# DaviGuanabara/dronechase

Measured on AMD Instinct MI355X. Metric: env-steps/sec (whole job), random-action rollout, higher is better.
Workload: dtype f32

## Files before the change

dronechase_amd/csrc/te_engage.hpp:

```cpp
#pragma once
#include "te_logic.hpp"
#include "te_stacked.hpp"
#include <type_traits>

namespace te {

#if defined(TE_DEBUG_STAMPS) && !defined(TE_NO_ESTAMP)
#define TE_ESTAMP(idx, wait)                                                                                   \
  do {                                                                                                         \
    if (wait) asm volatile("s_waitcnt vmcnt(0) lgkmcnt(0)" ::: "memory");                                      \
    if (p.dbg && threadIdx.x == 0) p.dbg[64 + blockIdx.x * 16 + (idx)] = __builtin_amdgcn_s_memrealtime();     \
  } while (0)
#else
#define TE_ESTAMP(idx, wait) do {} while (0)
#endif

template <class V> TE_DEV void plan_slot_l4(uint16_t* __restrict__ items, int dense_min, int lane, int s, bool a, uint64_t& dense, int& n, uint64_t& live) {
  const unsigned long long b = __ballot(a);
  const int cnt = __popcll(b);
  if (cnt == 0) return;
  live |= (uint64_t)1 << s;
  if (s == 0 || cnt >= dense_min || n + cnt > kMixedCap) { dense |= (uint64_t)1 << s; return; }
  if (a) items[n + (int)__builtin_amdgcn_mbcnt_hi((uint32_t)(b >> 32), __builtin_amdgcn_mbcnt_lo((uint32_t)b, 0u))] = (uint16_t)(lane | (s << 8));
  n += cnt;
// ... 137 lines not shown
    }
    if (invader || reset) st(TE_D_NAV_STATE, s, (uint32_t)TE_NAV_WAIT);
    return respawn;
  }
};

template <int DM>
TE_DEV void drone_contact_pass(const Params& p, int env, bool valid, uint64_t A) {
  const te_config& c = p.cfg;
  const int D = p.D;
  const EnvIO io(p, env);
  float qx[DM], qy[DM], qz[DM], ux[DM], uy[DM], uz[DM];
  uint64_t moved = 0u;
#pragma unroll
  for (int s = 0; s < DM; ++s) {
    qx[s] = qy[s] = qz[s] = ux[s] = uy[s] = uz[s] = 0.0f;
    if (s < D) {
      qx[s] = io.ldf(TE_D_POS, s); qy[s] = io.ldf(TE_D_POS + 1, s); qz[s] = io.ldf(TE_D_POS + 2, s);
      ux[s] = io.ldf(TE_D_VEL, s); uy[s] = io.ldf(TE_D_VEL + 1, s); uz[s] = io.ldf(TE_D_VEL + 2, s);
    }
  }
  const float two_r = 2.0f * c.contact_radius;
#pragma unroll
  for (int i = 0; i < DM; ++i) {
#pragma unroll
    for (int j = i + 1; j < DM; ++j) {
      float nx = qx[j] - qx[i], ny = qy[j] - qy[i], nz = qz[j] - qz[i];
      const float d = sqrtf(nx * nx + ny * ny + nz * nz);
      const bool hit = valid && ((A >> i) & (A >> j) & 1u) != 0u && d < two_r && d > 0.0f;
      const float inv = hit ? 1.0f / d : 0.0f;
      nx *= inv; ny *= inv; nz *= inv;
      const float push = hit ? 0.5f * (two_r - d) : 0.0f;
      const float vn = (ux[j] - ux[i]) * nx + (uy[j] - uy[i]) * ny + (uz[j] - uz[i]) * nz;
      const float dv = (hit && vn < 0.0f) ? 0.5f * vn : 0.0f;
      qx[i] -= push * nx; qy[i] -= push * ny; qz[i] -= push * nz; qx[j] += push * nx; qy[j] += push * ny; qz[j] += push * nz;
      ux[i] += dv * nx; uy[i] += dv * ny; uz[i] += dv * nz; ux[j] -= dv * nx; uy[j] -= dv * ny; uz[j] -= dv * nz;
      moved |= hit ? (((uint64_t)1 << i) | ((uint64_t)1 << j)) : (uint64_t)0;
    }
  }
#pragma unroll
  for (int s = 0; s < DM; ++s) {
    if ((moved >> s) & 1u) {
      io.stf(TE_D_POS, s, qx[s]); io.stf(TE_D_POS + 1, s, qy[s]); io.stf(TE_D_POS + 2, s, qz[s]);
      io.stf(TE_D_VEL, s, ux[s]); io.stf(TE_D_VEL + 1, s, uy[s]); io.stf(TE_D_VEL + 2, s, uz[s]);
    }
  }
}

template <int PM, int IM, bool CONTACT = false>
__global__ __launch_bounds__(64) void engage_kernel(Params p, const float* __restrict__ actions, StepOut o) {
  TE_EXACT
  constexpr int DM = PM + IM;
  using M = typename std::conditional<(DM > 32), uint64_t, uint32_t>::type;
  constexpr M one = 1;
  auto popc = [](M m) { return sizeof(M) == 8 ? __popcll((unsigned long long)m) : __popc((uint32_t)m); };
  auto lowest = [](M m) { return sizeof(M) == 8 ? __ffsll((long long)m) - 1 : __ffs((int)(uint32_t)m) - 1; };
  __shared__ float xs[DM][4];
  __shared__ float rows[64 * TE_OBS_INERTIAL_WORDS];
  const te_config& c = p.cfg;
  const int D = p.D, P = c.n_pursuers;
  const int lane = threadIdx.x;
  const int env = blockIdx.x * 64 + lane;
  const bool valid = env < p.N;
  const GView g{p.dstate, p.estate, D, p.Npad, env, P};
  TE_ESTAMP(0, 0);
  const M pur_bits = (one << P) - one, all_bits = D >= (int)(8 * sizeof(M)) ? ~(M)0 : ((one << D) - one), inv_bits = all_bits & ~pur_bits;
  const bool scripted = all_scripted(c);

  const __amdgpu_buffer_rsrc_t rd = __builtin_amdgcn_make_buffer_rsrc(p.dstate, 0, (int)((uint32_t)(TE_DRONE_WORDS + TE_X_WORDS) * (uint32_t)D * (uint32_t)p.Npad * 4u), 0x00020000);
  const __amdgpu_buffer_rsrc_t re = __builtin_amdgcn_make_buffer_rsrc(p.estate, 0, (int)((uint32_t)TE_ENV_WORDS * (uint32_t)p.Npad * 4u), 0x00020000);
  const int voff = env * 4;
  const uint32_t plane = (uint32_t)p.Npad * 4u;
  auto ld = [&](int w, int s) { return __builtin_amdgcn_raw_buffer_load_b32(rd, voff, (int)(((uint32_t)w * (uint32_t)D + (uint32_t)s) * plane), 0); };
  auto le = [&](int w) { return __builtin_amdgcn_raw_buffer_load_b32(re, voff, (int)((uint32_t)w * plane), 0); };
  auto st = [&](int w, int s, uint32_t v) { __builtin_amdgcn_raw_buffer_store_b32(v, rd, voff, (int)(((uint32_t)w * (uint32_t)D + (uint32_t)s) * plane), 0); };
  auto stf = [&](int w, int s, float v) { st(w, s, __float_as_uint(v)); };
  auto stv = [&](int w, int slot_off, uint32_t v) { __builtin_amdgcn_raw_buffer_store_b32(v, rd, slot_off, (int)((uint32_t)w * (uint32_t)D * plane), 0); };
  auto ste = [&](int w, uint32_t v) { __builtin_amdgcn_raw_buffer_store_b32(v, re, voff, (int)((uint32_t)w * plane), 0); };
  auto stef = [&](int w, float v) { ste(w, __float_as_uint(v)); };
  float px[DM], py[DM], pz[DM];
  uint32_t armed_w[DM];
  int mun[PM], lf[PM];
  float fx[PM], fy[PM], fz[PM];
  const uint32_t* __restrict__ lm32 = reinterpret_cast<const uint32_t*>(p.live_mask);
  const uint64_t live = (uint64_t)__builtin_amdgcn_readfirstlane(lm32[2 * blockIdx.x]) | ((uint64_t)__builtin_amdgcn_readfirstlane(lm32[2 * blockIdx.x + 1]) << 32);
#pragma unroll
  for (int s = 0; s < DM; ++s) {
    px[s] = py[s] = pz[s] = 0.0f; armed_w[s] = 0u;
    if (s < D && (s < P || ((live >> s) & 1u))) {
      px[s] = __uint_as_float(ld(TE_D_OBS_POS, s)); py[s] = __uint_as_float(ld(TE_D_OBS_POS + 1, s)); pz[s] = __uint_as_float(ld(TE_D_OBS_POS + 2, s));
      armed_w[s] = ld(TE_D_ARMED, s);
    }
  }
#pragma unroll
  for (int q = 0; q < PM; ++q) {
    mun[q] = 0; lf[q] = 0; fx[q] = fy[q] = fz[q] = 0.0f;
    if (q < P) {
      mun[q] = (int)ld(TE_D_MUNITION, q); lf[q] = (int)ld(TE_D_LAST_FIRED, q);
      fx[q] = __uint_as_float(ld(TE_D_FORMATION, q)); fy[q] = __uint_as_float(ld(TE_D_FORMATION + 1, q)); fz[q] = __uint_as_float(ld(TE_D_FORMATION + 2, q));
    }
  }
  float ag[9];
#pragma unroll
  for (int k = 0; k < 9; ++k) ag[k] = __uint_as_float(ld(TE_D_OBS_EULER + k, 0));
  uint32_t se[3][PM];
#pragma unroll
  for (int k = 0; k < 3; ++k)
#pragma unroll
    for (int q = 0; q < PM; ++q) se[k][q] = (p.snap && q < P) ? ld(TE_D_OBS_EULER + k, q) : 0u;
  int step = (int)le(TE_E_STEP) + 1;
  int max_step = (int)le(TE_E_MAX_STEP);
  int round = (int)le(TE_E_ROUND);
  const float last_dist = __uint_as_float(le(TE_E_LAST_DIST));
  int agent_kills = (int)le(TE_E_AGENT_KILLS), allies_kills = (int)le(TE_E_ALLIES_KILLS), deads = (int)le(TE_E_DEADS);
  uint32_t episode = le(TE_E_EPISODE);
  float4 act = make_float4(0.0f, 0.0f, 0.0f, 0.0f);
  if (valid) act = reinterpret_cast<const float4*>(actions)[env];

  TE_ESTAMP(1, 1);
  M S = 0, zone = 0, org = 0;
#pragma unroll
  for (int s = 0; s < DM; ++s) {
    const M a = (s < D && armed_w[s] != 0u && valid) ? one : (M)0;
    const float n = fnorm(V3{px[s], py[s], pz[s]});
    S |= a << s;
    zone |= (a & (n > c.dome_radius ? one : (M)0)) << s;
    org |= (a & (n < c.origin_range ? one : (M)0)) << s;
  }
  int tgt[PM]; float dmin[PM];
#pragma unroll
  for (int q = 0; q < PM; ++q) {
    tgt[q] = -1; dmin[q] = 0.0f;
#pragma unroll
    for (int j = 1; j < DM; ++j) {
      const float d = fdist(V3{px[q], py[q], pz[q]}, V3{px[j], py[j], pz[j]});
      const bool take = q < P && j >= P && ((S >> q) & (S >> j) & one) != 0 && (tgt[q] < 0 || d < dmin[q]);
      tgt[q] = take ? j : tgt[q];
      dmin[q] = take ? d : dmin[q];
    }
  }
  auto pos_of = [&](int s) {
    V3 r{0.0f, 0.0f, 0.0f};
#pragma unroll
    for (int k = 0; k < DM; ++k) if (k == s) r = V3{px[k], py[k], pz[k]};
    return r;
  };

  TE_ESTAMP(2, 0);
  M A = S;
  if (valid) {
    stef(TE_E_LAST_ACTION + 0, act.x); stef(TE_E_LAST_ACTION + 1, act.y); stef(TE_E_LAST_ACTION + 2, act.z); stef(TE_E_LAST_ACTION + 3, act.w);
    ste(TE_E_STEP, (uint32_t)step);
    ste(TE_E_SNAP_MASK, (uint32_t)S); ste(TE_E_SNAP_MASK_HI, (uint32_t)((uint64_t)S >> 32));
  }
  M killed = 0;
  auto kill = [&](int j) { killed |= one << j; A &= ~(one << j); };
  int agent_shots = 0, ally_shots = 0, exploded = 0, pursuer_suicided = 0, agent_suicided = 0;
#pragma unroll
  for (int q = 0; q < PM; ++q) {
    if (q < P && valid && ((S >> q) & one) && tgt[q] >= 0 && dmin[q] < c.shoot_range && gun_available(c, mun[q], lf[q], step) && mun[q] > 0) {
      mun[q] -= 1; lf[q] = step;
      st(TE_D_MUNITION, q, (uint32_t)mun[q]); st(TE_D_LAST_FIRED, q, (uint32_t)step);
      const U4 r = env_rng(c, env, RNG_HIT, (uint32_t)q, 0, episode, (uint32_t)step);
      if (u01(r.x) < c.hit_prob) {
        kill(tgt[q]);
        if (q == 0) agent_shots += 1; else ally_shots += 1;
        if (c.evaluation) g.si(TE_D_KILLS, q, g.gi(TE_D_KILLS, q) + 1);
      }
// ... 229 lines not shown
    unsigned long long sb = __ballot(task != 0u);
    for (; sb; sb &= sb - 1) {
      const int l = __ffsll((long long)sb) - 1;
      const uint32_t t = (uint32_t)__builtin_amdgcn_readlane((int)task, l);
      const uint32_t ep = (uint32_t)__builtin_amdgcn_readlane((int)episode, l);
      const M armed_l = (M)((uint64_t)(uint32_t)__builtin_amdgcn_readlane((int)(uint32_t)A, l) |
                            ((uint64_t)(uint32_t)__builtin_amdgcn_readlane((int)(uint32_t)((uint64_t)A >> 32), l) << 32));
      const bool reset = (t >> 8) != 0u;
      if (lane < D) {
        const GView gv{p.dstate, p.estate, D, p.Npad, (int)(blockIdx.x * 64 + l), P};
        V3 w{0.0f, 0.0f, 0.0f};
        const bool placed = spawn_slot_at(c, gv, lane, (int)(t & 0xFFu), ep, reset, ((armed_l >> lane) & one) != 0, w);
        xs[lane][0] = w.x; xs[lane][1] = w.y; xs[lane][2] = w.z; xs[lane][3] = placed ? 1.0f : 0.0f;
      }
      asm volatile("s_waitcnt lgkmcnt(0)" ::: "memory");
      if (lane == l) {
#pragma unroll
        for (int s = 0; s < DM; ++s)
          if (s < D && xs[s][3] != 0.0f) { px[s] = xs[s][0]; py[s] = xs[s][1]; pz[s] = xs[s][2]; }
        armed_post = snap_mask;
        if (reset) {
#pragma unroll
          for (int q = 0; q < PM; ++q)
            if (q < P) { mun[q] = max_munition_of(c, q); lf[q] = -c.cooldown_steps; fx[q] = px[q]; fy[q] = py[q]; fz[q] = pz[q]; }
        }
      }
      asm volatile("s_waitcnt lgkmcnt(0)" ::: "memory");
    }
  }
  TE_ESTAMP(7, 0);
  if (o.obs.inertial) {
    float row15[TE_OBS_INERTIAL_WORDS];
    inertial_row(row15, px[0], py[0], pz[0], ag, mun[0], lf[0], step);
#pragma unroll
    for (int k = 0; k < TE_OBS_INERTIAL_WORDS; ++k) rows[lane * TE_OBS_INERTIAL_WORDS + k] = row15[k];
    asm volatile("s_waitcnt lgkmcnt(0)" ::: "memory");
    const int n_out = min(64, p.N - (int)blockIdx.x * 64) * TE_OBS_INERTIAL_WORDS;
    float* dst = o.obs.inertial + (size_t)blockIdx.x * 64 * TE_OBS_INERTIAL_WORDS;
#pragma unroll
    for (int k = 0; k < TE_OBS_INERTIAL_WORDS; ++k)
      if (k * 64 + lane < n_out) dst[k * 64 + lane] = rows[k * 64 + lane];
  }
  if (valid && o.obs.last_action) reinterpret_cast<float4*>(o.obs.last_action)[env] = act;
  TE_ESTAMP(8, 0);
  if (valid) {
    int first_skipped = -1;
    if (!scripted && !(armed_post & one)) first_skipped = (armed_post & pur_bits & ~one) ? lowest(armed_post & pur_bits & ~one) : -1;
#pragma unroll
    for (int q = 0; q < PM; ++q) {
      if (q < P) {
        stf(TE_X_REF + 0, q, px[q]); stf(TE_X_REF + 1, q, py[q]); stf(TE_X_REF + 2, q, pz[q]);
        if ((q > 0 || scripted) && ((armed_post >> q) & one) && q != first_skipped) {
          float out[3] = {0.0f, 0.0f, 0.0f};
          const bool ext = driven_externally(c, q);
          if (!ext && c.ally_policy == TE_ALLY_BT) {
            const V3 me{px[q], py[q], pz[q]};
            if (gun_available(c, mun[q], lf[q], step)) {
              int t = -1; float bd = 0.0f; V3 tp{0.0f, 0.0f, 0.0f};
              if ((snap_mask >> q) & one) {
#pragma unroll
                for (int j = 1; j < DM; ++j) {
                  if (j >= P && ((snap_mask >> j) & one)) {
                    const V3 pj{px[j], py[j], pz[j]};
                    const float d = fdist(me, pj);
                    if (t < 0 || d < bd) { t = j; bd = d; tp = pj; }
                  }
                }
              }
              x_cmd_toward(me, tp, c.ally_speed, out);
            } else x_cmd_toward(me, V3{fx[q], fy[q], fz[q]}, c.ally_speed, out);
          } else if (ext || c.ally_policy != TE_ALLY_FROZEN) {
            out[0] = g.gf(TE_D_SETPOINT + 0, q); out[1] = g.gf(TE_D_SETPOINT + 1, q); out[2] = g.gf(TE_D_SETPOINT + 3, q);
          }
          stf(TE_X_CMD + 0, q, out[0]); stf(TE_X_CMD + 1, q, out[1]); stf(TE_X_CMD + 2, q, out[2]);
        }
      }
    }
  }
  TE_ESTAMP(9, 0);
  {
    uint64_t dense = 0u, live = 0u; int n = 0;
    uint16_t* items = p.mixed_items + (size_t)blockIdx.x * kMixedCap;
    for (int s = 0; s < D; ++s) plan_slot_l4<void>(items, p.dense_min, lane, s, valid && ((armed_post >> s) & one) != 0, dense, n, live);
    if (lane == 0) { p.slot_mask[blockIdx.x] = dense; p.mixed_count[blockIdx.x] = (uint32_t)n; p.live_mask[blockIdx.x] = live; }
  }
  TE_ESTAMP(10, 0);
  TE_ESTAMP(11, 1);
}

}

namespace te {

template <int DM>
TE_DEV uint32_t own_sphere_regs(const te_config& c, int D, const float (&px)[DM], const float (&py)[DM], const float (&pz)[DM], const float ag[9],
                                uint32_t A, uint32_t (&cell)[DM], float (&rhat)[DM]) {
  uint32_t owners = 0u;
  const V3 apos{px[0], py[0], pz[0]};
  const M3 R = x_inverse_attitude(ag[0], ag[1], ag[2]);
  cell[0] = 0u; rhat[0] = 1.0f;
#pragma unroll
  for (int j = 1; j < DM; ++j) {
    int cj; lidar_cell_fast(c, x_mul(R, sub(V3{px[j], py[j], pz[j]}, apos)), cj, rhat[j]);
    cell[j] = (uint32_t)cj;
    const bool in = j < D && ((A >> j) & 1u) != 0u;
    uint32_t same = 0u; float r_owner = 2.0f;
#pragma unroll
    for (int k = 1; k < j; ++k) {
      const bool hit = ((owners >> k) & 1u) != 0u && cell[k] == cell[j];
      same |= (hit ? 1u : 0u) << k;
      r_owner = hit ? rhat[k] : r_owner;
    }
    const bool wins = in && (same ? rhat[j] < r_owner : rhat[j] < 1.0f);
    owners = wins ? ((owners & ~same) | (1u << j)) : owners;
  }
  return owners;
}
template <int DM>
TE_DEV void record_sphere_regs(const StepOut& o, int npad, int env, bool to_terminal, uint32_t owners, const uint32_t (&cell)[DM]) {
  if (!o.persist || !o.obs.lidar) return;
  uint16_t* pv = o.prev + env;
  int n = 0;
#pragma unroll
  for (int j = 1; j < DM; ++j)
    if (!to_terminal && ((owners >> j) & 1u)) { n += 1; pv[(size_t)n * npad] = (uint16_t)cell[j]; }
  pv[0] = (uint16_t)n;
}
template <int DM>
TE_DEV void patch_sphere_regs(const te_config& c, float* __restrict__ dst, int env, int P, uint32_t owners, const uint32_t (&cell)[DM], const float (&rhat)[DM]) {
  if (!dst) return;
  dst += (size_t)env * lidar_words(c);
  const bool time_plane = c.lidar_channels != 2;
#pragma unroll
  for (int j = 1; j < DM; ++j) if ((owners >> j) & 1u) dst[cell[j]] = rhat[j];
#pragma unroll
  for (int j = 1; j < DM; ++j) if ((owners >> j) & 1u) dst[TE_LIDAR_CELLS + cell[j]] = (float)(j < P ? TE_TYPE_LOYALWINGMAN : TE_TYPE_LOITERINGMUNITION) / 5.0f;
  if (time_plane) {
#pragma unroll
    for (int j = 1; j < DM; ++j) if ((owners >> j) & 1u) dst[2 * TE_LIDAR_CELLS + cell[j]] = 0.1f;
  }
}
TE_DEV void inertial_row_regs(const te_config& c, float* dst, float x, float y, float z, const float a9[9], int mu, int lfi, int st) {
  const float two_pi = 2.0f * kPi;
  dst[0] = clampf(x / c.dome_radius, -1.0f, 1.0f); dst[1] = clampf(y / c.dome_radius, -1.0f, 1.0f); dst[2] = clampf(z / c.dome_radius, -1.0f, 1.0f);
#pragma unroll
  for (int k = 0; k < 3; ++k) {
    dst[3 + k] = clampf(a9[3 + k] / c.max_speed, -1.0f, 1.0f);
    dst[6 + k] = clampf(a9[k] / kPi, -1.0f, 1.0f);
    dst[9 + k] = clampf(a9[6 + k] / two_pi, -1.0f, 1.0f);
  }
  float gs[3];
  gun_state(c, mu, lfi, st, max_munition_of(c, 0), gs);
  dst[12] = gs[0]; dst[13] = gs[1]; dst[14] = gs[2];
}
TE_DEV void write_rows_regs(const Params& p, const ObsOut& o, float (&rows)[64 * TE_OBS_INERTIAL_WORDS], int lane, bool valid, int env, const float row[TE_OBS_INERTIAL_WORDS], float4 act) {
  if (o.inertial) {
#pragma unroll
    for (int k = 0; k < TE_OBS_INERTIAL_WORDS; ++k) rows[lane * TE_OBS_INERTIAL_WORDS + k] = row[k];
    asm volatile("s_waitcnt lgkmcnt(0)" ::: "memory");
    const int n_out = min(64, p.N - (int)blockIdx.x * 64) * TE_OBS_INERTIAL_WORDS;
    float* dst = o.inertial + (size_t)blockIdx.x * 64 * TE_OBS_INERTIAL_WORDS;
#pragma unroll
    for (int k = 0; k < TE_OBS_INERTIAL_WORDS; ++k)
      if (k * 64 + lane < n_out) dst[k * 64 + lane] = rows[k * 64 + lane];
  }
  if (valid && o.last_action) reinterpret_cast<float4*>(o.last_action)[env] = act;
}
// ... 78 lines not shown
        if (u01(r.x) < c.hit_prob) { killed |= 1u << tgt[q]; shots += 1; }
      }
    }
  }
#pragma unroll
  for (int q = 0; q < PM; ++q)
    if (q < P && valid && ((S >> q) & 1u) && tgt[q] >= 0 && dmin[q] < c.explosion_range) { killed |= (1u << q) | (1u << tgt[q]); exploded += 1; }
  A &= ~killed;
  for (uint32_t m = killed; m; m &= m - 1) io.disarm(__ffs(m) - 1);
  kills += shots; deads += exploded;
  float gs[3];
  gun_state(c, mun[0], lf[0], step, max_munition_of(c, 0), gs);
  const bool ready = gs[2] == 1.0f || gs[0] == 0.0f;
  float bonus = 0.0f, penalty = 0.0f;
  const float score = ready ? -cur : cur * (2.0f * gs[1] - 1.0f);
  if (0.01f < last - cur && ready) bonus += c.approach_bonus_gain * fnorm(V3{ag[3], ag[4], ag[5]});
  bonus += 1000.0f * (float)shots; penalty += 1000.0f * (float)exploded;
  const bool outside_p = (zone & pur_bits) != 0u, outside_i = (zone & inv_bits) != 0u;
  if (outside_p) penalty += 1000.0f;
  const float reward = score + bonus - penalty;
  const bool term = step > max_step || outside_p || outside_i || __popc(A & pur_bits) < P;
  const bool to_terminal = valid && term && c.auto_reset;
  if (valid) {
    io.ste(TE_E_AGENT_KILLS, (uint32_t)kills); io.ste(TE_E_DEADS, (uint32_t)deads);
    o.reward[env] = reward; o.done[env] = term ? 1 : 0;
    reinterpret_cast<int4*>(o.info)[env] = make_int4(kills, 0, deads, 0);
  }
  uint32_t cell[DM]; float rhat[DM];
  const uint32_t owners = own_sphere_regs<DM>(c, D, px, py, pz, ag, A, cell, rhat);
  float row[TE_OBS_INERTIAL_WORDS];
  if (to_terminal) {
    inertial_row_regs(c, row, px[0], py[0], pz[0], ag, mun[0], lf[0], step);
    if (o.term.inertial) { for (int k = 0; k < TE_OBS_INERTIAL_WORDS; ++k) o.term.inertial[(size_t)env * TE_OBS_INERTIAL_WORDS + k] = row[k]; }
    if (o.term.last_action) reinterpret_cast<float4*>(o.term.last_action)[env] = act;
  }
  terminal_tiles(c, o.term.lidar, to_terminal, lane);
  if (valid) { patch_sphere_regs<DM>(c, to_terminal ? o.term.lidar : o.obs.lidar, env, P, owners, cell, rhat); record_sphere_regs<DM>(o, p.Npad, env, to_terminal, owners, cell); }
  auto set_pos = [&](int s, V3 w) {
#pragma unroll
    for (int k = 0; k < DM; ++k) if (k == s) { px[k] = w.x; py[k] = w.y; pz[k] = w.z; }
  };
  if (valid) {
    for (uint32_t m = inv_bits & ~A; m; m &= m - 1) {
      const int j = __ffs(m) - 1;
      const V3 w = stage02_invader_position(c, env, j, episode, (uint32_t)step);
      io.respawn(c, j, w); set_pos(j, w);
    }
    A |= inv_bits;
    io.stef(TE_E_PREV_SNAP_MIN, cur); io.stef(TE_E_LAST_DIST, cur);
  }
  if (to_terminal) {
    episode += 1u; step = 0;
    io.ste(TE_E_EPISODE, episode); io.ste(TE_E_STEP, 0u); io.ste(TE_E_MAX_STEP, (uint32_t)c.max_step); io.ste(TE_E_ROUND, 0u);
    io.ste(TE_E_AGENT_KILLS, 0u); io.ste(TE_E_ALLIES_KILLS, 0u); io.ste(TE_E_DEADS, 0u);
#pragma unroll
    for (int k = 0; k < 4; ++k) io.ste(TE_E_LAST_ACTION + k, 0u);
    for (int j = P; j < D; ++j) { const V3 w = stage02_invader_position(c, env, j, episode, 0u); io.respawn(c, j, w); set_pos(j, w); }
    for (int q = 0; q < P; ++q) {
      const U4 r = env_rng(c, env, RNG_SPAWN_PURSUER, (uint32_t)q, 0, episode, 0);
      const V3 w = stage02_position(c.pursuer_spawn_radius, 0.0f, u01(r.x), u01(r.y), u01(r.z));
      io.respawn(c, q, w); set_pos(q, w);
    }
#pragma unroll
    for (int q = 0; q < PM; ++q) if (q < P) { mun[q] = max_munition_of(c, q); lf[q] = -c.cooldown_steps; }
    A = all_bits;
    io.ste(TE_E_SNAP_MASK, A);
    float d0 = 0.0f; bool any = false;
#pragma unroll
    for (int j = 1; j < DM; ++j) {
      const float d = fdist(V3{px[0], py[0], pz[0]}, V3{px[j], py[j], pz[j]});
      const bool take = j >= P && j < D && (!any || d < d0);
      d0 = take ? d : d0; any = any || take;
    }
    io.stef(TE_E_PREV_SNAP_MIN, d0); io.stef(TE_E_LAST_DIST, d0);
    act = make_float4(0.0f, 0.0f, 0.0f, 0.0f);
#pragma unroll
    for (int k = 0; k < 9; ++k) ag[k] = 0.0f;
  }
  inertial_row_regs(c, row, px[0], py[0], pz[0], ag, mun[0], lf[0], step);
  write_rows_regs(p, o.obs, rows, lane, valid, env, row, act);
  {
    uint64_t dense = 0u;
    for (int s = 0; s < D; ++s) if (__ballot(valid && ((A >> s) & 1u))) dense |= (uint64_t)1 << s;
    if (lane == 0) { p.slot_mask[blockIdx.x] = dense; p.mixed_count[blockIdx.x] = 0u; p.live_mask[blockIdx.x] = dense; }
  }
}

__global__ __launch_bounds__(64) void engage_stage01_kernel(Params p, const float* __restrict__ actions, StepOut o) {
  constexpr int DM = 3;
  __shared__ float rows[64 * TE_OBS_INERTIAL_WORDS];
  const te_config& c = p.cfg;
  const int lane = threadIdx.x, env = blockIdx.x * 64 + lane;
  const bool valid = env < p.N;
  const EnvIO io(p, env);
  const GView g{p.dstate, p.estate, 3, p.Npad, env, 2};
  float px[DM], py[DM], pz[DM]; uint32_t A = 0u;
#pragma unroll
  for (int s = 0; s < DM; ++s) {
    px[s] = io.ldf(TE_D_OBS_POS, s); py[s] = io.ldf(TE_D_OBS_POS + 1, s); pz[s] = io.ldf(TE_D_OBS_POS + 2, s);
    A |= (io.ld(TE_D_ARMED, s) != 0u && valid ? 1u : 0u) << s;
  }
  int mun0 = (int)io.ld(TE_D_MUNITION, 0), lf0 = (int)io.ld(TE_D_LAST_FIRED, 0);
  float ag[9];
#pragma unroll
  for (int k = 0; k < 9; ++k) ag[k] = io.ldf(TE_D_OBS_EULER + k, 0);
  int step = (int)io.le(TE_E_STEP) + 1;
  const int max_step = (int)io.le(TE_E_MAX_STEP);
  int kills = (int)io.le(TE_E_AGENT_KILLS);
  uint32_t episode = io.le(TE_E_EPISODE);
  const float last = __uint_as_float(io.le(TE_E_LAST_DIST));
  float4 act = make_float4(0.0f, 0.0f, 0.0f, 0.0f);
  if (valid) act = reinterpret_cast<const float4*>(actions)[env];
  if (valid) {
    io.stef(TE_E_LAST_ACTION + 0, act.x); io.stef(TE_E_LAST_ACTION + 1, act.y); io.stef(TE_E_LAST_ACTION + 2, act.z); io.stef(TE_E_LAST_ACTION + 3, act.w);
    io.ste(TE_E_STEP, (uint32_t)step);
  }
  const V3 pp{px[0], py[0], pz[0]}, pi{px[2], py[2], pz[2]};
  const float d = dist(pi, pp);
  float bonus = 0.0f, penalty = 0.0f;
  if (d < last) bonus += c.approach_bonus_gain * norm(V3{ag[3], ag[4], ag[5]});
  const bool caught = d < c.catch_distance;
  if (caught) bonus += 1000.0f;
  if (d > c.dome_radius) penalty += 1000.0f;
  const float reward = -d + bonus - penalty;
  const bool term = step > max_step || norm(pp) > c.dome_radius || norm(pi) > c.dome_radius;
  const bool to_terminal = valid && term && c.auto_reset;
  kills += caught ? 1 : 0;
  if (valid) {
    o.reward[env] = reward; o.done[env] = term ? 1 : 0;
    reinterpret_cast<int4*>(o.info)[env] = make_int4(kills, 0, 0, 0);
  }
  uint32_t cell[DM]; float rhat[DM];
  const uint32_t owners = own_sphere_regs<DM>(c, 3, px, py, pz, ag, A, cell, rhat);
  float row[TE_OBS_INERTIAL_WORDS];
  if (to_terminal) {
    inertial_row_regs(c, row, px[0], py[0], pz[0], ag, mun0, lf0, step);
    if (o.term.inertial) { for (int k = 0; k < TE_OBS_INERTIAL_WORDS; ++k) o.term.inertial[(size_t)env * TE_OBS_INERTIAL_WORDS + k] = row[k]; }
    if (o.term.last_action) reinterpret_cast<float4*>(o.term.last_action)[env] = act;
  }
  terminal_tiles(c, o.term.lidar, to_terminal, lane);
  if (valid) { patch_sphere_regs<DM>(c, to_terminal ? o.term.lidar : o.obs.lidar, env, 2, owners, cell, rhat); record_sphere_regs<DM>(o, p.Npad, env, to_terminal, owners, cell); }
  if (valid) {
    V3 p2 = pi;
    if (caught) {
      p2 = stage01_cube(c, env, RNG_RESPAWN, 2, episode, (uint32_t)step);
      stage01_replace_invader(c, g, p2, episode, (uint32_t)step);
      io.ste(TE_E_AGENT_KILLS, (uint32_t)kills);
      px[2] = p2.x; py[2] = p2.y; pz[2] = p2.z;
    }
    io.stef(TE_E_LAST_DIST, dist(p2, pp));
  }
  if (to_terminal) {
    stage01_reset_env(c, g);
    episode += 1u; step = 0;
    const V3 n0 = stage01_cube(c, env, RNG_SPAWN_PURSUER, 0, episode, 0);
    px[0] = n0.x; py[0] = n0.y; pz[0] = n0.z;
    mun0 = 0; lf0 = (A & 1u) ? lf0 : -c.cooldown_steps;
    A = 7u;
    act = make_float4(0.0f, 0.0f, 0.0f, 0.0f);
#pragma unroll
    for (int k = 0; k < 9; ++k) ag[k] = 0.0f;
  }
  inertial_row_regs(c, row, px[0], py[0], pz[0], ag, mun0, lf0, step);
  write_rows_regs(p, o.obs, rows, lane, valid, env, row, act);
  {
    uint64_t dense = 0u;
    for (int s = 0; s < 3; ++s) if (__ballot(valid && ((A >> s) & 1u))) dense |= (uint64_t)1 << s;
    if (lane == 0) { p.slot_mask[blockIdx.x] = dense; p.mixed_count[blockIdx.x] = 0u; p.live_mask[blockIdx.x] = dense; }
  }
}

}
```

dronechase_amd/csrc/te_engage_slots.hpp:

```cpp
#pragma once
#include "te_engage.hpp"

namespace te {

constexpr int kSlotWaves = 16;
constexpr int kSlotPursuers = 4;

struct SlotRows {
  int D, P;
  TE_DEV int accS() const { return 0; }
  TE_DEV int accZone() const { return 1; }
  TE_DEV int accOrg() const { return 2; }
  TE_DEV int accOwn() const { return 3; }
  TE_DEV int pos(int k, int s) const { return 4 + k * D + s; }
  TE_DEV int cellr(int s) const { return 4 + 3 * D + 2 * s; }
  TE_DEV int npos(int k, int s) const { return 4 + (5 + k) * D + s; }
  TE_DEV int prec(int q) const { return 4 + 8 * D + q; }
  TE_DEV int prec2(int q) const { return 4 + 8 * D + 2 * q; }
};
__host__ __device__ inline int slot_lds_rows(int D, int P) { return 4 + 8 * D + 2 * P; }
enum : uint32_t { SLOT_HIT = 1u << 8, SLOT_EXPLODE = 1u << 9, SLOT_SUICIDE = 1u << 10 };

#define TE_SLOT_BARRIER() asm volatile("s_waitcnt lgkmcnt(0)\n\ts_barrier" ::: "memory")
#if defined(TE_DEBUG_STAMPS)
#define TE_WSTAMP(idx, wait)                                                                                              \
  do {                                                                                                                    \
    if (wait) asm volatile("s_waitcnt vmcnt(0) lgkmcnt(0)" ::: "memory");                                                 \
    if (p.dbg && s < 2 && lane == 0) p.dbg[64 + blockIdx.x * 16 + s * 8 + (idx)] = __builtin_amdgcn_s_memrealtime();     \
  } while (0)
#else
#define TE_WSTAMP(idx, wait) do {} while (0)
#endif

template <int DM>
__global__ __launch_bounds__(DM * 64) __attribute__((amdgpu_waves_per_eu(6, 10))) void engage_slots_kernel(Params p, const float* __restrict__ actions, StepOut o) {
  TE_EXACT
  extern __shared__ uint32_t sm[];
  const te_config& c = p.cfg;
  const int D = p.D, P = c.n_pursuers;
  const SlotRows R{D, P};
  const int lane = threadIdx.x & 63;
  const int s = __builtin_amdgcn_readfirstlane((int)(threadIdx.x >> 6));
  const int env = blockIdx.x * 64 + lane;
  const bool valid = env < p.N;
  const GView g{p.dstate, p.estate, D, p.Npad, env, P};
  const EnvIO io(p, env);
  const uint32_t pur_bits = (1u << P) - 1u, all_bits = (1u << D) - 1u, inv_bits = all_bits & ~pur_bits;
  const bool scripted = all_scripted(c);
  const bool is_p = s < P;
  auto L = [&](int row) -> uint32_t& { return sm[row * 64 + lane]; };
  auto Lf = [&](int row) { return __uint_as_float(sm[row * 64 + lane]); };
  auto Lor = [&](int row, uint32_t v) { __hip_atomic_fetch_or(&sm[row * 64 + lane], v, __ATOMIC_RELAXED, __HIP_MEMORY_SCOPE_WORKGROUP); };
  TE_WSTAMP(0, 0);

  const uint32_t* __restrict__ lm32 = reinterpret_cast<const uint32_t*>(p.live_mask);
  const uint32_t live = (uint32_t)__builtin_amdgcn_readfirstlane(lm32[2 * blockIdx.x]) & all_bits;
  const bool mine_live = is_p || ((live >> s) & 1u);
  auto next_round_of = [&](int r) { return r + (r < c.n_rounds ? 1 : c.n_rounds); };
  auto may_be_spawned = [&](int slot, int r) { const int i = slot - P; return i < invaders_in_round(c, next_round_of(r)) || i < invaders_in_round(c, 1); };
  if (!mine_live) {
    const int r = (int)io.le(TE_E_ROUND);
    if (__ballot(valid && may_be_spawned(s, r)) == 0ull) return;
  }
  float mx = io.ldf(TE_D_OBS_POS, s), my = io.ldf(TE_D_OBS_POS + 1, s), mz = io.ldf(TE_D_OBS_POS + 2, s);
  const uint32_t marmed_w = io.ld(TE_D_ARMED, s);
  const V3 apos{io.ldf(TE_D_OBS_POS, 0), io.ldf(TE_D_OBS_POS + 1, 0), io.ldf(TE_D_OBS_POS + 2, 0)};
  float ag[9];
#pragma unroll
  for (int k = 0; k < 3; ++k) ag[k] = io.ldf(TE_D_OBS_EULER + k, 0);
#pragma unroll
  for (int k = 3; k < 9; ++k) ag[k] = 0.0f;
  const uint32_t w_step = io.le(TE_E_STEP), w_max_step = io.le(TE_E_MAX_STEP), w_round = io.le(TE_E_ROUND), w_episode = io.le(TE_E_EPISODE);
  uint32_t w_last_dist = 0u, w_ak = 0u, w_lk = 0u, w_dd = 0u;
  float4 act = make_float4(0.0f, 0.0f, 0.0f, 0.0f);
  if (s == 0) {
#pragma unroll
    for (int k = 3; k < 9; ++k) ag[k] = io.ldf(TE_D_OBS_EULER + k, 0);
    w_last_dist = io.le(TE_E_LAST_DIST); w_ak = io.le(TE_E_AGENT_KILLS); w_lk = io.le(TE_E_ALLIES_KILLS); w_dd = io.le(TE_E_DEADS);
    if (valid) act = reinterpret_cast<const float4*>(actions)[env];
  }
  uint32_t w_mun = 0u, w_lf = 0u; float fx = 0.0f, fy = 0.0f, fz = 0.0f;
  if (is_p) {
    w_mun = io.ld(TE_D_MUNITION, s); w_lf = io.ld(TE_D_LAST_FIRED, s);
    fx = io.ldf(TE_D_FORMATION, s); fy = io.ldf(TE_D_FORMATION + 1, s); fz = io.ldf(TE_D_FORMATION + 2, s);
  }
  uint32_t zero = 0u;
  asm volatile("" : "+s"(zero));
  if (s == 0) { L(R.accS()) = 0u; L(R.accZone()) = 0u; L(R.accOrg()) = 0u; L(R.accOwn()) = 0u; }
  TE_SLOT_BARRIER();
  int step = (int)w_step + 1;
  int max_step = (int)w_max_step, round = (int)w_round;
  uint32_t episode = w_episode;
  int mun = (int)w_mun, lf = (int)w_lf;
  const float last_dist = __uint_as_float(w_last_dist);
  int agent_kills = (int)w_ak, allies_kills = (int)w_lk, deads = (int)w_dd;
  if (!mine_live) { mx = my = mz = 0.0f; }
  TE_WSTAMP(1, 1);

  const uint32_t a_me = (mine_live && marmed_w != zero && valid) ? 1u : 0u;
  {
    const float n = fnorm(V3{mx, my, mz});
    Lor(R.accS(), a_me << s); Lor(R.accZone(), (a_me & (n > c.dome_radius ? 1u : 0u)) << s); Lor(R.accOrg(), (a_me & (n < c.origin_range ? 1u : 0u)) << s);
    L(R.pos(0, s)) = __float_as_uint(mx); L(R.pos(1, s)) = __float_as_uint(my); L(R.pos(2, s)) = __float_as_uint(mz);
  }
  int cj = 0; float rh = 1.0f;
  if (s >= 1) {
    const M3 Rm = x_inverse_attitude(ag[0], ag[1], ag[2]);
    lidar_cell_fast(c, x_mul(Rm, sub(V3{mx, my, mz}, apos)), cj, rh);
    *reinterpret_cast<uint2*>(&sm[R.cellr(s) * 64 + 2 * lane]) = make_uint2((uint32_t)cj, __float_as_uint(rh));
  }
  TE_WSTAMP(2, 0);
  TE_SLOT_BARRIER();
  TE_WSTAMP(3, 0);
  const uint32_t S = L(R.accS()), zone = L(R.accZone()), org = L(R.accOrg());
  if (is_p) {
    int tgt = -1; float dmin = 0.0f;
    for (uint32_t m = live & inv_bits; m; m &= m - 1u) {
      const int j = __ffs((int)m) - 1;
      const float d = fdist(V3{mx, my, mz}, V3{Lf(R.pos(0, j)), Lf(R.pos(1, j)), Lf(R.pos(2, j))});
      const bool take = a_me != 0u && ((S >> j) & 1u) != 0u && (tgt < 0 || d < dmin);
      tgt = take ? j : tgt;
      dmin = take ? d : dmin;
    }
    uint32_t rec = (uint32_t)(tgt + 1);
    if (a_me && tgt >= 0 && dmin < c.shoot_range && gun_available(c, mun, lf, step) && mun > 0) {
      mun -= 1; lf = step;
      io.st(TE_D_MUNITION, s, (uint32_t)mun); io.st(TE_D_LAST_FIRED, s, (uint32_t)step);
      const U4 r = env_rng(c, env, RNG_HIT, (uint32_t)s, 0, episode, (uint32_t)step);
      if (u01(r.x) < c.hit_prob) {
        rec |= SLOT_HIT;
        if (c.evaluation) g.si(TE_D_KILLS, s, g.gi(TE_D_KILLS, s) + 1);
      }
    }
    if (a_me && tgt >= 0 && dmin < c.explosion_range) rec |= SLOT_EXPLODE | (mun == 0 ? SLOT_SUICIDE : 0u);
    L(R.prec(s)) = rec;
  }
  TE_SLOT_BARRIER();

  uint32_t killed = 0u;
  int agent_shots = 0, ally_shots = 0, exploded = 0, pursuer_suicided = 0, agent_suicided = 0;
  for (int q = 0; q < P; ++q) {
    const uint32_t r = L(R.prec(q));
    const int t = (int)(r & 0xFFu) - 1;
    if (r & SLOT_HIT) { killed |= 1u << t; if (q == 0) agent_shots += 1; else ally_shots += 1; }
    if (r & SLOT_EXPLODE) {
      killed |= (1u << q) | (1u << t);
      if ((r & SLOT_SUICIDE) && q == 0) agent_suicided += 1;
      else if (r & SLOT_SUICIDE) pursuer_suicided += 1;
      else exploded += 1;
    }
  }
  if ((!c.evaluation || (c.evaluation & TE_EVAL_ORIGIN_RULE)) && valid) killed |= org & inv_bits;
  const uint32_t A = S & ~killed;
  if ((killed >> s) & 1u) io.disarm(s);
  if (agent_shots + ally_shots > 0) max_step += c.step_increment;
  const int armed_invaders = __popc(A & inv_bits), armed_pursuers = __popc(A & pur_bits);
  const bool all_rounds_over = armed_invaders == 0 && round >= c.n_rounds;
  bool term;
  if (c.evaluation) term = (c.max_step > 0 && step > max_step) || all_rounds_over || zone != 0u || armed_pursuers == 0;
  else term = step > max_step || all_rounds_over || zone != 0u || armed_pursuers == 0 || (c.agent_death_terminates && !(A & 1u)) || apos.z < -5.99f;
  const bool to_terminal = valid && term && c.auto_reset;
  bool own = false;
  if (s >= 1) {
    own = ((A >> s) & 1u) != 0u && rh < 1.0f;
    for (uint32_t m = live & ~1u & ~(1u << s); m; m &= m - 1u) {
      const int k = __ffs((int)m) - 1;
      const uint2 cr = *reinterpret_cast<const uint2*>(&sm[R.cellr(k) * 64 + 2 * lane]);
      const float rk = __uint_as_float(cr.y);
      const bool beaten = ((A >> k) & 1u) != 0u && cr.x == (uint32_t)cj && (rk < rh || (rk == rh && k < s));
      own = own && !beaten;
    }
    if (own && valid) Lor(R.accOwn(), 1u << s);
  }
  const float flag_me = (float)(s < P ? TE_TYPE_LOYALWINGMAN : TE_TYPE_LOITERINGMUNITION) / 5.0f;
  const bool time_plane = c.lidar_channels != 2;
  auto patch = [&](float* dst) {
    dst += (size_t)env * lidar_words(c);
    dst[cj] = rh; dst[TE_LIDAR_CELLS + cj] = flag_me;
    if (time_plane) dst[2 * TE_LIDAR_CELLS + cj] = 0.1f;
  };
  if (valid && own && !to_terminal && o.obs.lidar) patch(o.obs.lidar);
  const unsigned long long term_b = __ballot(to_terminal);
  if (o.term.lidar && term_b && is_p) {
    for (unsigned long long tb = term_b; tb; tb &= tb - 1) {
      const int l = __ffsll((long long)tb) - 1;
      float* tile = o.term.lidar + (size_t)(blockIdx.x * 64 + l) * lidar_words(c);
      for (int e = s * 64 + lane; e < lidar_words(c); e += 64 * P) tile[e] = 1.0f;
    }
  }

  auto pos_of = [&](int t) { return V3{__uint_as_float(sm[R.pos(0, t) * 64 + lane]), __uint_as_float(sm[R.pos(1, t) * 64 + lane]), __uint_as_float(sm[R.pos(2, t) * 64 + lane])}; };
  if (s == 0) {
    if (valid) {
      io.stef(TE_E_LAST_ACTION + 0, act.x); io.stef(TE_E_LAST_ACTION + 1, act.y); io.stef(TE_E_LAST_ACTION + 2, act.z); io.stef(TE_E_LAST_ACTION + 3, act.w);
      io.ste(TE_E_STEP, (uint32_t)step);
      io.ste(TE_E_SNAP_MASK, S); io.ste(TE_E_SNAP_MASK_HI, 0u);
    }
    agent_kills += agent_shots; allies_kills += ally_shots; deads += exploded;
    if (to_terminal) {
      if (o.term.inertial) inertial_row_regs(c, o.term.inertial + (size_t)env * TE_OBS_INERTIAL_WORDS, mx, my, mz, ag, mun, lf, step);
      if (o.term.last_action) reinterpret_cast<float4*>(o.term.last_action)[env] = act;
    }
    float reward = 0.0f, cur_dist = last_dist;
    if (!c.evaluation) {
      float gs[3];
      gun_state(c, mun, lf, step, max_munition_of(c, 0), gs);
      const float dist_origin = fnorm(apos);
      int ally = -1;
      if ((S & 1u) && __popc(S & pur_bits) > 1) {
        float bd = 0.0f;
        for (int a = 1; a < P; ++a) {
          if ((S >> a) & 1u) {
            const float d = fdist(pos_of(a), apos);
            if (ally < 0 || d < bd) { ally = a; bd = d; }
          }
        }
      }
      const int chooser = ally < 0 ? 0 : ally;
      const int target = ((S >> chooser) & 1u) ? (int)(sm[R.prec(chooser) * 64 + lane] & 0xFFu) - 1 : -1;
      const V3 tp = target >= 0 ? pos_of(target) : V3{0.0f, 0.0f, 0.0f};
      cur_dist = fdist(apos, tp);
      const bool ready = gs[2] == 1.0f || gs[0] == 0.0f;
      float bonus = 0.0f, penalty = 0.0f;
      if (0.01f < last_dist - cur_dist && ready) bonus += c.approach_bonus_gain * fnorm(V3{ag[3], ag[4], ag[5]});
      const float score = ready ? -cur_dist : cur_dist * (2.0f * gs[1] - 1.0f);
      if (agent_shots > 0 || agent_suicided > 0) bonus += (float)(agent_shots + agent_suicided) * 1000.0f;
      if (ally_shots > 0 || pursuer_suicided > 0) bonus += 0.5f * (float)(ally_shots + pursuer_suicided) * 1000.0f;
      else if (exploded > 0) penalty += 1000.0f * (float)exploded;
      if (apos.z < -5.0f) penalty += (-5.0f - apos.z) * 1000.0f;
      if (zone & pur_bits) penalty += 1000.0f;
      if (dist_origin > c.born_radius - 2.0f) penalty += dist_origin - c.born_radius - 2.0f;
      reward = score + bonus - penalty;
    }
    if (valid) {
      if (!c.evaluation) io.stef(TE_E_LAST_DIST, cur_dist);
      io.ste(TE_E_AGENT_KILLS, (uint32_t)agent_kills); io.ste(TE_E_ALLIES_KILLS, (uint32_t)allies_kills); io.ste(TE_E_DEADS, (uint32_t)deads);
      if (agent_shots + ally_shots > 0) io.ste(TE_E_MAX_STEP, (uint32_t)max_step);
      o.reward[env] = reward;
      o.done[env] = term ? 1 : 0;
      reinterpret_cast<int4*>(o.info)[env] = make_int4(agent_kills, allies_kills, deads, round);
      io.ste(TE_E_INFO_WAVE, (uint32_t)round);
    }
  }

  uint32_t task = 0u;
  uint32_t snap_mask = S;
  auto mask_after_spawn = [&](int rnd, bool reset) {
    const uint32_t m = reset ? pur_bits : (A & pur_bits);
    const int n = invaders_in_round(c, rnd);
    return (uint32_t)(m | ((((1u << n) - 1u) << P) & all_bits));
  };
  if (valid && !term && armed_invaders == 0 && armed_pursuers > 0) {
    round = round + (round < c.n_rounds ? 1 : c.n_rounds);
    snap_mask = mask_after_spawn(round, false);
    if (s == 0) { io.ste(TE_E_ROUND, (uint32_t)round); io.ste(TE_E_SNAP_MASK, snap_mask); io.ste(TE_E_SNAP_MASK_HI, 0u); }
    task = (uint32_t)round;
  }
  if (to_terminal) {
    episode += 1u; step = 0; max_step = c.max_step; round = 1;
    snap_mask = mask_after_spawn(1, true);
    if (s == 0) {
      io.ste(TE_E_EPISODE, episode); io.ste(TE_E_STEP, 0u); io.ste(TE_E_MAX_STEP, (uint32_t)c.max_step); io.ste(TE_E_ROUND, 1u); io.ste(TE_E_INFO_WAVE, 1u);
      io.ste(TE_E_AGENT_KILLS, 0u); io.ste(TE_E_ALLIES_KILLS, 0u); io.ste(TE_E_DEADS, 0u);
      if (c.reward_model != TE_REWARD_L5_C1) io.stef(TE_E_LAST_DIST, c.dome_radius);
#pragma unroll
      for (int k = 0; k < 4; ++k) io.ste(TE_E_LAST_ACTION + k, 0u);
      io.ste(TE_E_SNAP_MASK, snap_mask); io.ste(TE_E_SNAP_MASK_HI, 0u);
    }
    act = make_float4(0.0f, 0.0f, 0.0f, 0.0f);
#pragma unroll
    for (int k = 0; k < 9; ++k) ag[k] = 0.0f;
    task = 1u | (1u << 8);
  }
  if (task != 0u) {
    const bool reset = (task >> 8) != 0u;
    V3 w{0.0f, 0.0f, 0.0f};
    const bool placed = io.spawn_uniform(c, env, s, (int)(task & 0xFFu), episode, reset, ((A >> s) & 1u) != 0u, w);
    if (placed) { mx = w.x; my = w.y; mz = w.z; }
    if (reset && is_p) { mun = max_munition_of(c, s); lf = -c.cooldown_steps; fx = mx; fy = my; fz = mz; }
  }
  if (s == 0 && __ballot(task != 0u) != 0ull) {
    for (uint32_t m = inv_bits & ~live; m; m &= m - 1u) {
      const int k2 = __ffs((int)m) - 1;
      if (__ballot(valid && may_be_spawned(k2, (int)w_round)) != 0ull) continue;
      if (task != 0u) io.st(TE_D_NAV_STATE, k2, (uint32_t)TE_NAV_WAIT);
    }
  }
  const uint32_t armed_post = task != 0u ? snap_mask : A;
  L(R.npos(0, s)) = __float_as_uint(mx); L(R.npos(1, s)) = __float_as_uint(my); L(R.npos(2, s)) = __float_as_uint(mz);
  if (o.term.lidar && term_b) asm volatile("s_waitcnt vmcnt(0)" ::: "memory");
  TE_WSTAMP(4, 0);
  TE_SLOT_BARRIER();
  TE_WSTAMP(5, 0);

  if (s >= 1 && to_terminal && own && o.term.lidar) patch(o.term.lidar);
  if (o.persist && o.obs.lidar && valid) {
    const uint32_t owners = L(R.accOwn());
    uint16_t* pv = o.prev + env;
    if (s == 0) pv[0] = (uint16_t)(to_terminal ? 0 : __popc(owners));
    else if (own && !to_terminal) pv[(size_t)(__popc(owners & ((1u << s) - 1u)) + 1) * p.Npad] = (uint16_t)cj;
  }
  if (s == 0) {
    if (o.obs.inertial && valid) inertial_row_regs(c, o.obs.inertial + (size_t)env * TE_OBS_INERTIAL_WORDS, mx, my, mz, ag, mun, lf, step);
    if (valid && o.obs.last_action) reinterpret_cast<float4*>(o.obs.last_action)[env] = act;
  }
  if (is_p && valid) {
    int first_skipped = -1;
    if (!scripted && !(armed_post & 1u)) first_skipped = (armed_post & pur_bits & ~1u) ? __ffs((int)(armed_post & pur_bits & ~1u)) - 1 : -1;
    io.stf(TE_X_REF + 0, s, mx); io.stf(TE_X_REF + 1, s, my); io.stf(TE_X_REF + 2, s, mz);
    if ((s > 0 || scripted) && ((armed_post >> s) & 1u) && s != first_skipped) {
      float out[3] = {0.0f, 0.0f, 0.0f};
      const bool ext = driven_externally(c, s);
      if (!ext && c.ally_policy == TE_ALLY_BT) {
        const V3 me{mx, my, mz};
        if (gun_available(c, mun, lf, step)) {
          int t = -1; float bd = 0.0f; V3 tp{0.0f, 0.0f, 0.0f};
          if ((snap_mask >> s) & 1u) {
            for (int j = P; j < D; ++j) {
              if (__ballot((snap_mask >> j) & 1u) == 0ull) continue;
              if ((snap_mask >> j) & 1u) {
                const V3 pj{Lf(R.npos(0, j)), Lf(R.npos(1, j)), Lf(R.npos(2, j))};
                const float d = fdist(me, pj);
                if (t < 0 || d < bd) { t = j; bd = d; tp = pj; }
              }
            }
          }
          x_cmd_toward(me, tp, c.ally_speed, out);
        } else x_cmd_toward(me, V3{fx, fy, fz}, c.ally_speed, out);
      } else if (ext || c.ally_policy != TE_ALLY_FROZEN) {
        out[0] = g.gf(TE_D_SETPOINT + 0, s); out[1] = g.gf(TE_D_SETPOINT + 1, s); out[2] = g.gf(TE_D_SETPOINT + 3, s);
      }
      io.stf(TE_X_CMD + 0, s, out[0]); io.stf(TE_X_CMD + 1, s, out[1]); io.stf(TE_X_CMD + 2, s, out[2]);
    }
  }
  const int writer = 0;
  if (s >= 1 || s == writer) {
    uint64_t dense = 0u, livem = 0u; int n = 0;
    uint16_t* items = p.mixed_items + (size_t)blockIdx.x * kMixedCap;
    const int k_last = s == writer ? D - 1 : s;
    for (int k = 0; k <= k_last; ++k) {
      const bool a = valid && ((armed_post >> k) & 1u) != 0u;
      const unsigned long long b = __ballot(a);
      const int cnt = __popcll(b);
      if (cnt == 0) continue;
      livem |= (uint64_t)1 << k;
      if (k == 0 || cnt >= p.dense_min || n + cnt > kMixedCap) { dense |= (uint64_t)1 << k; continue; }
      if (k == s && a) items[n + (int)__builtin_amdgcn_mbcnt_hi((uint32_t)(b >> 32), __builtin_amdgcn_mbcnt_lo((uint32_t)b, 0u))] = (uint16_t)(lane | (k << 8));
      n += cnt;
    }
    if (s == writer && lane == 0) { p.slot_mask[blockIdx.x] = dense; p.mixed_count[blockIdx.x] = (uint32_t)n; p.live_mask[blockIdx.x] = livem; }
  }
  TE_WSTAMP(6, 0);
  TE_WSTAMP(7, 1);
}

struct MultiSlotRows {
  int D, P, H;
  TE_DEV int accS(int h = 0) const { return h; }
  TE_DEV int accZone(int h = 0) const { return H + h; }
  TE_DEV int accOrg(int h = 0) const { return 2 * H + h; }
  TE_DEV int pos(int k, int s) const { return 3 * H + k * D + s; }
  TE_DEV int npos(int k, int s) const { return 3 * H + (3 + k) * D + s; }
  TE_DEV int prec(int q) const { return 3 * H + 6 * D + q; }
  TE_DEV int accOwn() const { return 3 * H + 6 * D + P; }
  TE_DEV int cellr(int s) const { return 3 * H + 1 + 6 * D + P + 2 * s; }
};
__host__ __device__ inline int multi_slot_lds_rows(int D, int P, bool lidar) { return 3 * (D > 32 ? 2 : 1) + 6 * D + P + (lidar ? 1 + 2 * D : 0); }

template <int SPW, bool LIDAR, bool WIDE = false>
__global__ __launch_bounds__(1024) __attribute__((amdgpu_waves_per_eu(SPW == 1 ? 4 : 6))) void engage_slots_multi_kernel(Params p, const float* __restrict__ actions, StepOut o) {
  TE_EXACT
  extern __shared__ uint32_t sm[];
  const te_config& c = p.cfg;
  const int D = p.D, P = c.n_pursuers;
  const int W = (int)(blockDim.x >> 6);
  using M = typename std::conditional<WIDE, uint64_t, uint32_t>::type;
  constexpr M one = 1;
  constexpr int kSh = WIDE ? 63 : 31;
  static_assert(!(WIDE && LIDAR), "the own sphere's owner row is 32 bits");
  const MultiSlotRows R{D, P, WIDE ? 2 : 1};
  auto popcM = [](M m) { return WIDE ? __popcll((unsigned long long)m) : __popc((uint32_t)m); };
  auto ffsM = [](M m) { return WIDE ? __ffsll((long long)m) - 1 : __ffs((int)(uint32_t)m) - 1; };
  const int lane = threadIdx.x & 63;
  const int s = __builtin_amdgcn_readfirstlane((int)(threadIdx.x >> 6));
  const int env = blockIdx.x * 64 + lane;
  const bool valid = env < p.N;
  const GView g{p.dstate, p.estate, D, p.Npad, env, P};
  const EnvIO io(p, env);
  const M pur_bits = (one << P) - one, all_bits = D >= (int)(8 * sizeof(M)) ? ~(M)0 : (one << D) - one, inv_bits = all_bits & ~pur_bits;
  const bool scripted = all_scripted(c);
  const bool is_p = s < P;
  int sl[SPW]; bool has[SPW];
#pragma unroll
  for (int u = 0; u < SPW; ++u) { sl[u] = s + u * W; has[u] = sl[u] < D; }
  auto L = [&](int row) -> uint32_t& { return sm[row * 64 + lane]; };
  auto Lf = [&](int row) { return __uint_as_float(sm[row * 64 + lane]); };
  auto Lor = [&](int row, uint32_t v) { __hip_atomic_fetch_or(&sm[row * 64 + lane], v, __ATOMIC_RELAXED, __HIP_MEMORY_SCOPE_WORKGROUP); };
  TE_WSTAMP(0, 0);

  const uint32_t* __restrict__ lm32 = reinterpret_cast<const uint32_t*>(p.live_mask);
  const M live = (WIDE ? (M)((uint64_t)(uint32_t)__builtin_amdgcn_readfirstlane(lm32[2 * blockIdx.x]) | ((uint64_t)(uint32_t)__builtin_amdgcn_readfirstlane(lm32[2 * blockIdx.x + 1]) << 32))
                       : (M)(uint32_t)__builtin_amdgcn_readfirstlane(lm32[2 * blockIdx.x])) & all_bits;
  auto next_round_of = [&](int r) { return r + (r < c.n_rounds ? 1 : c.n_rounds); };
  auto may_be_spawned = [&](int slot, int r) { const int i = slot - P; return i < invaders_in_round(c, next_round_of(r)) || i < invaders_in_round(c, 1); };
  bool mine_live[SPW]; bool any_live = is_p;
#pragma unroll
  for (int u = 0; u < SPW; ++u) { mine_live[u] = has[u] && ((u == 0 && is_p) || ((live >> (sl[u] & kSh)) & one) != 0); any_live = any_live || mine_live[u]; }
  if (!any_live) {
    const int r = (int)io.le(TE_E_ROUND);
    bool maybe = false;
#pragma unroll
    for (int u = 0; u < SPW; ++u) maybe = maybe || (has[u] && may_be_spawned(sl[u], r));
    if (__ballot(valid && maybe) == 0ull) return;
  }
  float mx[SPW], my[SPW], mz[SPW]; uint32_t marmed_w[SPW];
#pragma unroll
  for (int u = 0; u < SPW; ++u) {
    const int ls = has[u] ? sl[u] : s;
    mx[u] = io.ldf(TE_D_OBS_POS, ls); my[u] = io.ldf(TE_D_OBS_POS + 1, ls); mz[u] = io.ldf(TE_D_OBS_POS + 2, ls);
    marmed_w[u] = io.ld(TE_D_ARMED, ls);
  }
  const uint32_t w_step = io.le(TE_E_STEP), w_max_step = io.le(TE_E_MAX_STEP), w_round = io.le(TE_E_ROUND), w_episode = io.le(TE_E_EPISODE);
  float ag[9];
#pragma unroll
  for (int k = 0; k < 9; ++k) ag[k] = 0.0f;
  V3 apos0{0.0f, 0.0f, 0.0f};
  if (LIDAR) {
#pragma unroll
    for (int k = 0; k < 3; ++k) ag[k] = io.ldf(TE_D_OBS_EULER + k, 0);
    apos0 = V3{io.ldf(TE_D_OBS_POS, 0), io.ldf(TE_D_OBS_POS + 1, 0), io.ldf(TE_D_OBS_POS + 2, 0)};
  }
  uint32_t w_last_dist = 0u, w_ak = 0u, w_lk = 0u, w_dd = 0u;
  float4 act = make_float4(0.0f, 0.0f, 0.0f, 0.0f);
  if (s == 0) {
#pragma unroll
    for (int k = LIDAR ? 3 : 0; k < 9; ++k) ag[k] = io.ldf(TE_D_OBS_EULER + k, 0);
    w_last_dist = io.le(TE_E_LAST_DIST); w_ak = io.le(TE_E_AGENT_KILLS); w_lk = io.le(TE_E_ALLIES_KILLS); w_dd = io.le(TE_E_DEADS);
    if (valid) act = reinterpret_cast<const float4*>(actions)[env];
  }
  uint32_t w_mun = 0u, w_lf = 0u, eul[3] = {0u, 0u, 0u}; float fx = 0.0f, fy = 0.0f, fz = 0.0f;
  if (is_p) {
    w_mun = io.ld(TE_D_MUNITION, s); w_lf = io.ld(TE_D_LAST_FIRED, s);
    fx = io.ldf(TE_D_FORMATION, s); fy = io.ldf(TE_D_FORMATION + 1, s); fz = io.ldf(TE_D_FORMATION + 2, s);
#pragma unroll
    for (int k = 0; k < 3; ++k) eul[k] = io.ld(TE_D_OBS_EULER + k, s);
  }
  uint32_t zero = 0u;
  asm volatile("" : "+s"(zero));
  if (s == 0) {
#pragma unroll
    for (int h = 0; h < (WIDE ? 2 : 1); ++h) { L(R.accS(h)) = 0u; L(R.accZone(h)) = 0u; L(R.accOrg(h)) = 0u; }
    if (LIDAR) L(R.accOwn()) = 0u;
  }
  TE_SLOT_BARRIER();
  int step = (int)w_step + 1;
  int max_step = (int)w_max_step, round = (int)w_round;
  uint32_t episode = w_episode;
  int mun = (int)w_mun, lf = (int)w_lf;
  const float last_dist = __uint_as_float(w_last_dist);
  int agent_kills = (int)w_ak, allies_kills = (int)w_lk, deads = (int)w_dd;
  TE_WSTAMP(1, 1);

  uint32_t a_me[SPW];
#pragma unroll
  for (int u = 0; u < SPW; ++u) {
    if (!mine_live[u]) { mx[u] = my[u] = mz[u] = 0.0f; }
    a_me[u] = (mine_live[u] && marmed_w[u] != zero && valid) ? 1u : 0u;
    if (has[u]) {
      const float n = fnorm(V3{mx[u], my[u], mz[u]});
      const int sh = sl[u] & 31, hh = WIDE ? (sl[u] >> 5) & 1 : 0;
      Lor(R.accS(hh), a_me[u] << sh); Lor(R.accZone(hh), (a_me[u] & (n > c.dome_radius ? 1u : 0u)) << sh); Lor(R.accOrg(hh), (a_me[u] & (n < c.origin_range ? 1u : 0u)) << sh);
      L(R.pos(0, sl[u])) = __float_as_uint(mx[u]); L(R.pos(1, sl[u])) = __float_as_uint(my[u]); L(R.pos(2, sl[u])) = __float_as_uint(mz[u]);
    }
  }
  int cj[SPW]; float rh[SPW];
#pragma unroll
  for (int u = 0; u < SPW; ++u) { cj[u] = 0; rh[u] = 1.0f; }
  if (LIDAR) {
    const M3 Rm = x_inverse_attitude(ag[0], ag[1], ag[2]);
#pragma unroll
    for (int u = 0; u < SPW; ++u) {
      if (has[u] && sl[u] >= 1) {
        lidar_cell_fast(c, x_mul(Rm, sub(V3{mx[u], my[u], mz[u]}, apos0)), cj[u], rh[u]);
        *reinterpret_cast<uint2*>(&sm[R.cellr(sl[u]) * 64 + 2 * lane]) = make_uint2((uint32_t)cj[u], __float_as_uint(rh[u]));
      }
    }
  }
  TE_WSTAMP(2, 0);
  TE_SLOT_BARRIER();
  TE_WSTAMP(3, 0);
  auto rdM = [&](int lo, int hi) { return WIDE ? (M)((uint64_t)L(lo) | ((uint64_t)L(hi) << 32)) : (M)L(lo); };
  const M S = rdM(R.accS(0), R.accS(1)), zone = rdM(R.accZone(0), R.accZone(1)), org = rdM(R.accOrg(0), R.accOrg(1));
  const V3 apos{Lf(R.pos(0, 0)), Lf(R.pos(1, 0)), Lf(R.pos(2, 0))};
  if (is_p) {
    int tgt = -1; float dmin = 0.0f;
    for (M m = live & inv_bits; m; m &= m - one) {
// ... 151 lines not shown
        if (zone & pur_bits) penalty += 1000.0f;
        if (dist_origin > c.born_radius - 2.0f) penalty += fminf(dist_origin - (c.born_radius - 2.0f), 1000.0f);
        reward = clampf(score + bonus - penalty, -3000.0f, 3000.0f);
      } else if (c.reward_model == TE_REWARD_L5_C1) {
        const int t1 = (S & one) ? (int)(sm[R.prec(0) * 64 + lane] & 0xFFu) - 1 : -1;
        const float d1 = t1 >= 0 ? fdist(apos, pos_of(t1)) : dist_origin;
        const float first = last_dist == 0.0f ? d1 : last_dist;
        float r1 = d1 < first ? c.approach_bonus_gain * fnorm(V3{ag[3], ag[4], ag[5]}) : 0.0f;
        if (agent_shots > 0) r1 += (float)agent_shots * 1000.0f;
        if (agent_suicided > 0) r1 -= 2.0f * (float)agent_suicided * 1000.0f;
        reward = clampf(r1, -3000.0f, 3000.0f);
        cur_dist = first;
      } else {
        if (0.01f < last_dist - cur_dist && ready) bonus += c.approach_bonus_gain * fnorm(V3{ag[3], ag[4], ag[5]});
        const float score = ready ? -cur_dist : cur_dist * (2.0f * gs[1] - 1.0f);
        if (agent_shots > 0 || agent_suicided > 0) bonus += (float)(agent_shots + agent_suicided) * 1000.0f;
        if (ally_shots > 0 || pursuer_suicided > 0) bonus += 0.5f * (float)(ally_shots + pursuer_suicided) * 1000.0f;
        else if (exploded > 0) penalty += 1000.0f * (float)exploded;
        if (apos.z < -5.0f) penalty += (-5.0f - apos.z) * 1000.0f;
        if (zone & pur_bits) penalty += 1000.0f;
        if (dist_origin > c.born_radius - 2.0f) penalty += dist_origin - c.born_radius - 2.0f;
        reward = score + bonus - penalty;
      }
    }
    if (valid) {
      if (!c.evaluation) io.stef(TE_E_LAST_DIST, cur_dist);
      io.ste(TE_E_AGENT_KILLS, (uint32_t)agent_kills); io.ste(TE_E_ALLIES_KILLS, (uint32_t)allies_kills); io.ste(TE_E_DEADS, (uint32_t)deads);
      if (agent_shots + ally_shots > 0) io.ste(TE_E_MAX_STEP, (uint32_t)max_step);
      o.reward[env] = reward;
      o.done[env] = term ? 1 : 0;
      reinterpret_cast<int4*>(o.info)[env] = make_int4(agent_kills, allies_kills, deads, round);
      io.ste(TE_E_INFO_WAVE, (uint32_t)round);
    }
  }

  uint32_t task = 0u;
  M snap_mask = S;
  auto mask_after_spawn = [&](int rnd, bool reset) {
    const M m = reset ? pur_bits : (A & pur_bits);
    const int n = invaders_in_round(c, rnd);
    return (M)(m | ((M)((((uint64_t)1 << n) - 1u) << P) & all_bits));
  };
  if (valid && !term && armed_invaders == 0 && armed_pursuers > 0) {
    round = round + (round < c.n_rounds ? 1 : c.n_rounds);
    snap_mask = mask_after_spawn(round, false);
    if (s == 0) { io.ste(TE_E_ROUND, (uint32_t)round); io.ste(TE_E_SNAP_MASK, (uint32_t)snap_mask); io.ste(TE_E_SNAP_MASK_HI, (uint32_t)((uint64_t)snap_mask >> 32)); }
    task = (uint32_t)round;
  }
  if (to_terminal) {
    episode += 1u; step = 0; max_step = c.max_step; round = 1;
    snap_mask = mask_after_spawn(1, true);
    if (s == 0) {
      io.ste(TE_E_EPISODE, episode); io.ste(TE_E_STEP, 0u); io.ste(TE_E_MAX_STEP, (uint32_t)c.max_step); io.ste(TE_E_ROUND, 1u); io.ste(TE_E_INFO_WAVE, 1u);
      io.ste(TE_E_AGENT_KILLS, 0u); io.ste(TE_E_ALLIES_KILLS, 0u); io.ste(TE_E_DEADS, 0u);
      if (c.reward_model != TE_REWARD_L5_C1) io.stef(TE_E_LAST_DIST, c.dome_radius);
#pragma unroll
      for (int k = 0; k < 4; ++k) io.ste(TE_E_LAST_ACTION + k, 0u);
      io.ste(TE_E_SNAP_MASK, (uint32_t)snap_mask); io.ste(TE_E_SNAP_MASK_HI, (uint32_t)((uint64_t)snap_mask >> 32));
    }
    act = make_float4(0.0f, 0.0f, 0.0f, 0.0f);
#pragma unroll
    for (int k = 0; k < 9; ++k) ag[k] = 0.0f;
    task = 1u | (1u << 8);
  }
  if (task != 0u) {
    const bool reset = (task >> 8) != 0u;
#pragma unroll
    for (int u = 0; u < SPW; ++u) {
      if (has[u]) {
        V3 w{0.0f, 0.0f, 0.0f};
        const bool placed = io.spawn_uniform(c, env, sl[u], (int)(task & 0xFFu), episode, reset, ((A >> (sl[u] & kSh)) & one) != 0, w);
        if (placed) { mx[u] = w.x; my[u] = w.y; mz[u] = w.z; }
      }
    }
    if (reset && is_p) { mun = max_munition_of(c, s); lf = -c.cooldown_steps; fx = mx[0]; fy = my[0]; fz = mz[0]; }
  }
  if (s == 0 && __ballot(task != 0u) != 0ull) {
    for (M m = inv_bits & ~live; m; m &= m - one) {
      const int k2 = ffsM(m);
      const int wv = k2 % W;
      bool stayed = wv < P;
      for (int u2 = 0; u2 < SPW && !stayed; ++u2) {
        const int s2 = wv + u2 * W;
        if (s2 < D) stayed = ((live >> s2) & one) != 0 || __ballot(valid && may_be_spawned(s2, (int)w_round)) != 0ull;
      }
      if (stayed) continue;
      if (task != 0u) io.st(TE_D_NAV_STATE, k2, (uint32_t)TE_NAV_WAIT);
    }
  }
  const M armed_post = task != 0u ? snap_mask : A;
#pragma unroll
  for (int u = 0; u < SPW; ++u)
    if (has[u]) { L(R.npos(0, sl[u])) = __float_as_uint(mx[u]); L(R.npos(1, sl[u])) = __float_as_uint(my[u]); L(R.npos(2, sl[u])) = __float_as_uint(mz[u]); }
  if (LIDAR && o.term.lidar && term_b) asm volatile("s_waitcnt vmcnt(0)" ::: "memory");
  TE_WSTAMP(4, 0);
  TE_SLOT_BARRIER();
  TE_WSTAMP(5, 0);

  if constexpr (LIDAR) {
    const uint32_t owners = L(R.accOwn());
#pragma unroll
    for (int u = 0; u < SPW; ++u) {
      if (has[u] && sl[u] >= 1) {
        if (to_terminal && own[u] && o.term.lidar) patch(o.term.lidar, cj[u], rh[u], sl[u]);
        if (o.persist && o.obs.lidar && valid && own[u] && !to_terminal)
          o.prev[env + (size_t)(__popc(owners & ((1u << (sl[u] & 31)) - 1u)) + 1) * p.Npad] = (uint16_t)cj[u];
      }
    }
    if (s == 0 && o.persist && o.obs.lidar && valid) o.prev[env] = (uint16_t)(to_terminal ? 0 : __popc(owners));
  }
  if (s == 0) {
    if (o.obs.inertial && valid) inertial_row_regs(c, o.obs.inertial + (size_t)env * TE_OBS_INERTIAL_WORDS, mx[0], my[0], mz[0], ag, mun, lf, step);
    if (valid && o.obs.last_action) reinterpret_cast<float4*>(o.obs.last_action)[env] = act;
  }
  if (is_p && valid) {
    int first_skipped = -1;
    if (!scripted && !(armed_post & one)) first_skipped = (armed_post & pur_bits & ~one) ? ffsM(armed_post & pur_bits & ~one) : -1;
    io.stf(TE_X_REF + 0, s, mx[0]); io.stf(TE_X_REF + 1, s, my[0]); io.stf(TE_X_REF + 2, s, mz[0]);
    if ((s > 0 || scripted) && ((armed_post >> s) & one) && s != first_skipped) {
      float out[3] = {0.0f, 0.0f, 0.0f};
      const bool ext = driven_externally(c, s);
      if (!ext && c.ally_policy == TE_ALLY_BT) {
        const V3 me{mx[0], my[0], mz[0]};
        if (gun_available(c, mun, lf, step)) {
          int t = -1; float bd = 0.0f; V3 tp{0.0f, 0.0f, 0.0f};
          if ((snap_mask >> s) & one) {
            for (int j = P; j < D; ++j) {
              if (__ballot(((snap_mask >> j) & one) != 0) == 0ull) continue;
              if ((snap_mask >> j) & one) {
                const V3 pj{Lf(R.npos(0, j)), Lf(R.npos(1, j)), Lf(R.npos(2, j))};
                const float d = fdist(me, pj);
                if (t < 0 || d < bd) { t = j; bd = d; tp = pj; }
              }
            }
          }
          x_cmd_toward(me, tp, c.ally_speed, out);
        } else x_cmd_toward(me, V3{fx, fy, fz}, c.ally_speed, out);
      } else if (ext || c.ally_policy != TE_ALLY_FROZEN) {
        out[0] = g.gf(TE_D_SETPOINT + 0, s); out[1] = g.gf(TE_D_SETPOINT + 1, s); out[2] = g.gf(TE_D_SETPOINT + 3, s);
      }
      io.stf(TE_X_CMD + 0, s, out[0]); io.stf(TE_X_CMD + 1, s, out[1]); io.stf(TE_X_CMD + 2, s, out[2]);
    }
  }
  {
    const int writer = 0;
    int top = s;
#pragma unroll
    for (int u = 1; u < SPW; ++u) if (has[u]) top = sl[u];
    uint64_t dense = 0u, livem = 0u; int n = 0;
    uint16_t* items = p.mixed_items + (size_t)blockIdx.x * kMixedCap;
    const int k_last = s == writer ? D - 1 : top;
    for (int k = 0; k <= k_last; ++k) {
      const bool a = valid && ((armed_post >> k) & one) != 0;
      const unsigned long long b = __ballot(a);
      const int cnt = __popcll(b);
      if (cnt == 0) continue;
      livem |= (uint64_t)1 << k;
      if (k == 0 || cnt >= p.dense_min || n + cnt > kMixedCap) { dense |= (uint64_t)1 << k; continue; }
      bool own = false;
#pragma unroll
      for (int u = 0; u < SPW; ++u) own = own || (has[u] && k == sl[u]);
      if (own && a) items[n + (int)__builtin_amdgcn_mbcnt_hi((uint32_t)(b >> 32), __builtin_amdgcn_mbcnt_lo((uint32_t)b, 0u))] = (uint16_t)(lane | (k << 8));
      n += cnt;
    }
    if (s == writer && lane == 0) { p.slot_mask[blockIdx.x] = dense; p.mixed_count[blockIdx.x] = (uint32_t)n; p.live_mask[blockIdx.x] = livem; }
  }
  TE_WSTAMP(6, 0);
  TE_WSTAMP(7, 1);
}

enum : uint32_t { SLOT2_KILL = 1u << 8 };

template <int DM>
__global__ __launch_bounds__(DM * 64) void engage_slots_stage02_kernel(Params p, const float* __restrict__ actions, StepOut o) {
  TE_EXACT
  extern __shared__ uint32_t sm[];
  const te_config& c = p.cfg;
  const int D = p.D, P = c.n_pursuers;
  const SlotRows R{D, P};
  const int lane = threadIdx.x & 63;
  const int s = __builtin_amdgcn_readfirstlane((int)(threadIdx.x >> 6));
  const int env = blockIdx.x * 64 + lane;
  const bool valid = env < p.N;
  const EnvIO io(p, env);
  const uint32_t pur_bits = (1u << P) - 1u, all_bits = (1u << D) - 1u, inv_bits = all_bits & ~pur_bits;
  const bool is_p = s < P;
  auto L = [&](int row) -> uint32_t& { return sm[row * 64 + lane]; };
  auto Lf = [&](int row) { return __uint_as_float(sm[row * 64 + lane]); };
  auto Lor = [&](int row, uint32_t v) { __hip_atomic_fetch_or(&sm[row * 64 + lane], v, __ATOMIC_RELAXED, __HIP_MEMORY_SCOPE_WORKGROUP); };

  float mx = io.ldf(TE_D_OBS_POS, s), my = io.ldf(TE_D_OBS_POS + 1, s), mz = io.ldf(TE_D_OBS_POS + 2, s);
  const uint32_t marmed_w = io.ld(TE_D_ARMED, s);
  const V3 apos{io.ldf(TE_D_OBS_POS, 0), io.ldf(TE_D_OBS_POS + 1, 0), io.ldf(TE_D_OBS_POS + 2, 0)};
  float ag[9];
#pragma unroll
  for (int k = 0; k < 3; ++k) ag[k] = io.ldf(TE_D_OBS_EULER + k, 0);
#pragma unroll
  for (int k = 3; k < 9; ++k) ag[k] = 0.0f;
  const uint32_t w_step = io.le(TE_E_STEP), w_max_step = io.le(TE_E_MAX_STEP), w_episode = io.le(TE_E_EPISODE);
  uint32_t w_kills = 0u, w_deads = 0u, w_last = 0u;
  float4 act = make_float4(0.0f, 0.0f, 0.0f, 0.0f);
  if (s == 0) {
#pragma unroll
    for (int k = 3; k < 9; ++k) ag[k] = io.ldf(TE_D_OBS_EULER + k, 0);
    w_kills = io.le(TE_E_AGENT_KILLS); w_deads = io.le(TE_E_DEADS); w_last = io.le(TE_E_PREV_SNAP_MIN);
    if (valid) act = reinterpret_cast<const float4*>(actions)[env];
  }
  uint32_t w_mun = 0u, w_lf = 0u;
  float qx[DM], qy[DM], qz[DM]; uint32_t qa[DM];
#pragma unroll
  for (int j = 0; j < DM; ++j) { qx[j] = qy[j] = qz[j] = 0.0f; qa[j] = 0u; }
  if (is_p) {
    w_mun = io.ld(TE_D_MUNITION, s); w_lf = io.ld(TE_D_LAST_FIRED, s);
#pragma unroll
    for (int j = 1; j < DM; ++j) {
      if ((inv_bits >> j) & 1u) {
        qx[j] = io.ldf(TE_D_OBS_POS, j); qy[j] = io.ldf(TE_D_OBS_POS + 1, j); qz[j] = io.ldf(TE_D_OBS_POS + 2, j); qa[j] = io.ld(TE_D_ARMED, j);
      }
    }
  }
  uint32_t zero = 0u;
  asm volatile("" : "+s"(zero));
  if (s == 0) { L(R.accS()) = 0u; L(R.accZone()) = 0u; L(R.accOrg()) = 0u; L(R.accOwn()) = 0u; }
  TE_SLOT_BARRIER();
  int step = (int)w_step + 1;
  const int max_step = (int)w_max_step;
  uint32_t episode = w_episode;
  int mun = (int)w_mun, lf = (int)w_lf;
  int kills = (int)w_kills, deads = (int)w_deads;
  const float last = __uint_as_float(w_last);

  const uint32_t a_me = (marmed_w != zero && valid) ? 1u : 0u;
  {
    const float n = fnorm(V3{mx, my, mz});
    Lor(R.accS(), a_me << s); Lor(R.accZone(), (a_me & (n > c.dome_radius ? 1u : 0u)) << s);
    L(R.pos(0, s)) = __float_as_uint(mx); L(R.pos(1, s)) = __float_as_uint(my); L(R.pos(2, s)) = __float_as_uint(mz);
  }
  int cj = 0; float rh = 1.0f;
  if (s >= 1) {
    const M3 Rm = x_inverse_attitude(ag[0], ag[1], ag[2]);
    lidar_cell_fast(c, x_mul(Rm, sub(V3{mx, my, mz}, apos)), cj, rh);
    *reinterpret_cast<uint2*>(&sm[R.cellr(s) * 64 + 2 * lane]) = make_uint2((uint32_t)cj, __float_as_uint(rh));
  }
  if (is_p) {
    int tgt = -1; float dmin = 0.0f;
#pragma unroll
    for (int j = 1; j < DM; ++j) {
      const float d = fdist(V3{mx, my, mz}, V3{qx[j], qy[j], qz[j]});
// ... 58 lines not shown
      const int l = __ffsll((long long)tb) - 1;
      float* tile = o.term.lidar + (size_t)(blockIdx.x * 64 + l) * lidar_words(c);
      for (int e = s * 64 + lane; e < lidar_words(c); e += 64 * D) tile[e] = 1.0f;
    }
  }
  if (s == 0) {
    if (valid) {
      io.stef(TE_E_LAST_ACTION + 0, act.x); io.stef(TE_E_LAST_ACTION + 1, act.y); io.stef(TE_E_LAST_ACTION + 2, act.z); io.stef(TE_E_LAST_ACTION + 3, act.w);
      io.ste(TE_E_STEP, (uint32_t)step); io.ste(TE_E_SNAP_MASK, S);
    }
    kills += shots; deads += exploded;
    float gs[3];
    gun_state(c, mun, lf, step, max_munition_of(c, 0), gs);
    const bool ready = gs[2] == 1.0f || gs[0] == 0.0f;
    float bonus = 0.0f, penalty = 0.0f;
    const float score = ready ? -cur : cur * (2.0f * gs[1] - 1.0f);
    if (0.01f < last - cur && ready) bonus += c.approach_bonus_gain * fnorm(V3{ag[3], ag[4], ag[5]});
    bonus += 1000.0f * (float)shots; penalty += 1000.0f * (float)exploded;
    if (outside_p) penalty += 1000.0f;
    const float reward = score + bonus - penalty;
    if (valid) {
      io.ste(TE_E_AGENT_KILLS, (uint32_t)kills); io.ste(TE_E_DEADS, (uint32_t)deads);
      o.reward[env] = reward; o.done[env] = term ? 1 : 0;
      reinterpret_cast<int4*>(o.info)[env] = make_int4(kills, 0, deads, 0);
    }
    if (to_terminal) {
      if (o.term.inertial) inertial_row_regs(c, o.term.inertial + (size_t)env * TE_OBS_INERTIAL_WORDS, mx, my, mz, ag, mun, lf, step);
      if (o.term.last_action) reinterpret_cast<float4*>(o.term.last_action)[env] = act;
    }
    if (valid) { io.stef(TE_E_PREV_SNAP_MIN, cur); io.stef(TE_E_LAST_DIST, cur); }
  }
  if (valid && !is_p && !((A >> s) & 1u)) {
    const V3 w = stage02_invader_position(c, env, s, episode, (uint32_t)step);
    io.respawn(c, s, w); mx = w.x; my = w.y; mz = w.z;
  }
  if (to_terminal) {
    episode += 1u; step = 0;
    if (s == 0) {
      io.ste(TE_E_EPISODE, episode); io.ste(TE_E_STEP, 0u); io.ste(TE_E_MAX_STEP, (uint32_t)c.max_step); io.ste(TE_E_ROUND, 0u);
      io.ste(TE_E_AGENT_KILLS, 0u); io.ste(TE_E_ALLIES_KILLS, 0u); io.ste(TE_E_DEADS, 0u);
#pragma unroll
      for (int k = 0; k < 4; ++k) io.ste(TE_E_LAST_ACTION + k, 0u);
      io.ste(TE_E_SNAP_MASK, all_bits);
    }
    V3 w;
    if (is_p) {
      const U4 r = env_rng(c, env, RNG_SPAWN_PURSUER, (uint32_t)s, 0, episode, 0);
      w = stage02_position(c.pursuer_spawn_radius, 0.0f, u01(r.x), u01(r.y), u01(r.z));
      mun = max_munition_of(c, s); lf = -c.cooldown_steps;
    } else w = stage02_invader_position(c, env, s, episode, 0u);
    io.respawn(c, s, w); mx = w.x; my = w.y; mz = w.z;
    act = make_float4(0.0f, 0.0f, 0.0f, 0.0f);
#pragma unroll
    for (int k = 0; k < 9; ++k) ag[k] = 0.0f;
  }
  L(R.npos(0, s)) = __float_as_uint(mx); L(R.npos(1, s)) = __float_as_uint(my); L(R.npos(2, s)) = __float_as_uint(mz);
  if (o.term.lidar && term_b) asm volatile("s_waitcnt vmcnt(0)" ::: "memory");
  TE_SLOT_BARRIER();

  if (s >= 1 && to_terminal && own && o.term.lidar) patch(o.term.lidar);
  if (o.persist && o.obs.lidar && valid) {
    const uint32_t owners = L(R.accOwn());
    uint16_t* pv = o.prev + env;
    if (s == 0) pv[0] = (uint16_t)(to_terminal ? 0 : __popc(owners));
    else if (own && !to_terminal) pv[(size_t)(__popc(owners & ((1u << s) - 1u)) + 1) * p.Npad] = (uint16_t)cj;
  }
  if (s == 0) {
    if (to_terminal) {
      float d0 = 0.0f; bool any = false;
      for (int j = P; j < D; ++j) {
        const float d = fdist(V3{mx, my, mz}, V3{Lf(R.npos(0, j)), Lf(R.npos(1, j)), Lf(R.npos(2, j))});
        const bool take = !any || d < d0;
        d0 = take ? d : d0; any = true;
      }
      io.stef(TE_E_PREV_SNAP_MIN, d0); io.stef(TE_E_LAST_DIST, d0);
    }
    if (o.obs.inertial && valid) inertial_row_regs(c, o.obs.inertial + (size_t)env * TE_OBS_INERTIAL_WORDS, mx, my, mz, ag, mun, lf, step);
    if (valid && o.obs.last_action) reinterpret_cast<float4*>(o.obs.last_action)[env] = act;
  }
  if (s == D - 1) {
    const uint32_t armed_post = to_terminal ? all_bits : ((A & pur_bits) | (valid ? inv_bits : 0u));
    uint64_t dense = 0u;
    for (int k = 0; k < D; ++k) if (__ballot(valid && ((armed_post >> k) & 1u))) dense |= (uint64_t)1 << k;
    if (lane == 0) { p.slot_mask[blockIdx.x] = dense; p.mixed_count[blockIdx.x] = 0u; p.live_mask[blockIdx.x] = dense; }
  }
}

}
```

dronechase_amd/csrc/te_env.hip:

```cpp
#include <hip/hip_runtime.h>
#include <hip/hip_ext.h>

#include <algorithm>
#include <cmath>
#include <cstdio>
#include <cstdlib>
#include <cstring>
#include <map>
#include <mutex>
#include <new>
#include <string>
#include <tuple>
#include <type_traits>
#include <vector>

#include "te_logic.hpp"
#include "te_stacked.hpp"
#include "te_stackview.hpp"
#include "te_engage.hpp"
#include "te_engage_slots.hpp"
#include "te_policy.hpp"
#include "te_wingman.hpp"
#include "te_policy_grad.hpp"
#include "te_policy_opt.hpp"
// ... 299 lines not shown
      const uint32_t stride = fill.n_fill_waves * 64u;
      for (uint32_t q = (uint32_t)wave * 64u + (uint32_t)lane; q < fill.total_quads; q += stride) TE_FILL_STORE(fill_dst + q);
      TE_K1_END(1);
      return;
    }
    wave -= (int)fill.n_fill_waves;
  }
  const int n_head = min(D, p.cfg.n_pursuers + 1) * nchunks;
  const int n_mixed = (FAMILY == FAM_LEVEL4 && p.dense_min > 1) ? kMixedWaves * nchunks : 0;
  if (wave >= n_head && wave < n_head + n_mixed) {
    wave -= n_head;
    const int m = wave / nchunks, chunk = wave - m * nchunks;
    const int count = __builtin_amdgcn_readfirstlane((int)((const uint32_t* __restrict__)p.mixed_count)[chunk]);
    if (m * 64 >= count) { TE_K1_END(0); return; }
    const int i = m * 64 + lane;
    const bool valid = i < count;
    const uint32_t item = valid ? (uint32_t)p.mixed_items[(size_t)chunk * kMixedCap + i] : 0u;
    if (HELP && role == 1) { noise_help<FAMILY, true>(p, (int)(item >> 8), chunk * 64 + (int)(item & 63u), valid, k1_lds, ready, 1u); return; }
    fly<FAMILY, NOISE, true, CES, HELP, HELP>(p, actions, (int)(item >> 8), chunk * 64 + (int)(item & 63u), valid, k1_lds, ready);
    TE_K1_END(3);
    return;
  }
  if (wave >= n_head) wave -= n_mixed;
  const int slot = wave / nchunks;
  const int chunk = wave - slot * nchunks;
  if (slot >= D) { TE_K1_END(0); return; }
  const uint32_t* __restrict__ sm32 = reinterpret_cast<const uint32_t*>(p.slot_mask);
  const uint32_t chunk_mask = __builtin_amdgcn_readfirstlane(sm32[2 * chunk + (slot >> 5)]);
  const int env = chunk * 64 + lane;
  if (HELP && FAMILY == FAM_LEVEL4) {
    const uint32_t gate = (chunk_mask >> (slot & 31)) & 1u;
    if (role == 1) { noise_help<FAMILY, true>(p, slot, env, env < p.N, k1_lds, ready, gate); return; }
    fly<FAMILY, NOISE, false, CES, true, true>(p, actions, slot, env, env < p.N, k1_lds, ready, gate);
    TE_K1_END(2);
    return;
  }
  if (!((chunk_mask >> (slot & 31)) & 1u)) { TE_K1_END(0); return; }
  if (HELP) {
    if (role == 1 && lane == 0) *ready = 0;
    asm volatile("s_waitcnt lgkmcnt(0)\n\ts_barrier" ::: "memory");
    if (role == 1) { noise_help<FAMILY, false>(p, slot, env, env < p.N, k1_lds, ready, 1u); return; }
  }
  fly<FAMILY, NOISE, false, CES, HELP>(p, actions, slot, env, env < p.N, k1_lds, ready);
  TE_K1_END(2);
}

template <int FAMILY>
__global__ __launch_bounds__(256) void reset_kernel(Params p, const uint8_t* __restrict__ mask) {
  int env = blockIdx.x * 256 + threadIdx.x;
  if (env >= p.N) return;
  if (mask && !mask[env]) return;
  GView v{p.dstate, p.estate, p.D, p.Npad, env, p.cfg.n_pursuers};
  reset_env<FAMILY>(p.cfg, v);
  if (p.ring)
    for (int k = 0; k < p.cfg.n_pursuers * TE_RING_DEPTH; ++k) p.ring[((size_t)env * p.cfg.n_pursuers * TE_RING_DEPTH + k) * (size_t)p.entry_words] = 0u;
}
__global__ __launch_bounds__(256) void snapshot_kernel(Params p) {
  const int env = blockIdx.x * 256 + threadIdx.x;
  if (env >= p.N) return;
  const GView v{p.dstate, p.estate, p.D, p.Npad, env, p.cfg.n_pursuers};
  const SnapRows sr{p.D, p.cfg.n_pursuers};
  for (int k = 0; k < 3; ++k) {
    for (int s = 0; s < p.D; ++s) p.snap[(size_t)(sr.pos() + k * p.D + s) * p.Npad + env] = (uint32_t)v.gi(TE_D_OBS_POS + k, s);
    for (int s = 0; s < sr.P; ++s) p.snap[(size_t)(sr.euler() + k * sr.P + s) * p.Npad + env] = (uint32_t)v.gi(TE_D_OBS_EULER + k, s);
  }
  p.snap[(size_t)sr.armed() * p.Npad + env] = armed_mask(v);
  p.snap[(size_t)sr.step() * p.Npad + env] = (uint32_t)v.egi(TE_E_STEP);
  p.snap[(size_t)sr.episode() * p.Npad + env] = (uint32_t)v.egi(TE_E_EPISODE);
  p.snap[(size_t)sr.done() * p.Npad + env] = 0u;
  uint32_t hi = 0u;
  for (int s = 32; s < p.D; ++s) hi |= (v.gi(TE_D_ARMED, s) ? 1u : 0u) << (s - 32);
  p.snap[(size_t)sr.armed_hi() * p.Npad + env] = hi;
}
template <int FAMILY>
TE_DEV void plan_slot(uint16_t* __restrict__ items, int dense_min, int lane, int s, bool a, uint64_t& dense, int& n, uint64_t& live) {
  const unsigned long long b = __ballot(a);
  const int cnt = __popcll(b);
  if (cnt == 0) return;
  live |= (uint64_t)1 << s;
  if (FAMILY != FAM_LEVEL4 || s == 0 || cnt >= dense_min || n + cnt > kMixedCap) { dense |= (uint64_t)1 << s; return; }
  if (a) items[n + (int)__builtin_amdgcn_mbcnt_hi((uint32_t)(b >> 32), __builtin_amdgcn_mbcnt_lo((uint32_t)b, 0u))] = (uint16_t)(lane | (s << 8));
  n += cnt;
}
TE_DEV void plan_done(const Params& p, int chunk, int lane, uint64_t dense, int n, uint64_t live) {
  if (lane == 0) { p.slot_mask[chunk] = dense; p.mixed_count[chunk] = (uint32_t)n; p.live_mask[chunk] = live; }
}
template <int FAMILY>
__global__ __launch_bounds__(64) void census_kernel(Params p) {
  const int chunk = blockIdx.x, l = threadIdx.x, env = chunk * 64 + l;
  uint64_t dense = 0u, live = 0u; int n = 0;
  uint16_t* items = p.mixed_items + (size_t)chunk * kMixedCap;
  for (int s = 0; s < p.D; ++s) plan_slot<FAMILY>(items, p.dense_min, l, s, env < p.N && p.dstate[((size_t)TE_D_ARMED * p.D + s) * p.Npad + env] != 0u, dense, n, live);
  plan_done(p, chunk, l, dense, n, live);
}
__global__ __launch_bounds__(256) void prepare_commands_kernel(Params p) {
  int env = blockIdx.x * 256 + threadIdx.x;
  if (env >= p.N) return;
  GView v{p.dstate, p.estate, p.D, p.Npad, env, p.cfg.n_pursuers};
  prepare_level4_commands(p.cfg, v);
}

static uint32_t staged_row_offset(const Params& p, const Rows& r, int row) {
  const int D = p.D;
  size_t w;
  if (row < r.munition()) {
    const int q = row / D, s = row - q * D;
    w = ((size_t)(q < 3 ? TE_D_OBS_POS + q : TE_D_ARMED) * D + s) * p.Npad;
  } else if (row < r.agent()) {
    const int k = row - r.munition();
    w = ((size_t)(k < r.P ? TE_D_MUNITION : TE_D_LAST_FIRED) * D + (k < r.P ? k : k - r.P)) * p.Npad;
  } else if (row < r.env()) w = ((size_t)(TE_D_OBS_EULER + (row - r.agent())) * D) * p.Npad;
  else return 0x80000000u | (uint32_t)((size_t)(row - r.env()) * p.Npad);
  return (uint32_t)w;
}
TE_DEV void stage_block(const Params& p, uint32_t* sm, const Rows& r, int env0) {
  const int lane = threadIdx.x & 63, nw = blockDim.x >> 6;
  const int wave = __builtin_amdgcn_readfirstlane((int)(threadIdx.x >> 6));
  const __amdgpu_buffer_rsrc_t rd = __builtin_amdgcn_make_buffer_rsrc(p.dstate, 0, (int)((uint32_t)(TE_DRONE_WORDS + TE_X_WORDS) * (uint32_t)p.D * (uint32_t)p.Npad * 4u), 0x00020000);
  const __amdgpu_buffer_rsrc_t re = __builtin_amdgcn_make_buffer_rsrc(p.estate, 0, (int)((uint32_t)TE_ENV_WORDS * (uint32_t)p.Npad * 4u), 0x00020000);
  const int voff = (env0 + lane) * 4;
  const uint32_t* __restrict__ tab = p.stage_tab;
  const int n = r.staged();
  constexpr int B = 32;
  for (int base = wave; base < n; base += B * nw) {
    uint32_t vals[B];
#pragma unroll
    for (int k = 0; k < B; ++k) {
      const int row = base + k * nw;
      vals[k] = 0u;
      if (row < n) {
        const uint32_t t = __builtin_amdgcn_readfirstlane(tab[row]);
        vals[k] = (t >> 31) ? __builtin_amdgcn_raw_buffer_load_b32(re, voff, (int)((t & 0x7FFFFFFFu) << 2), 0)
                            : __builtin_amdgcn_raw_buffer_load_b32(rd, voff, (int)(t << 2), 0);
      }
    }
#pragma unroll
    for (int k = 0; k < B; ++k) {
      const int row = base + k * nw;
      if (row < n) sm[row * kEPB + lane] = vals[k];
    }
  }
}

template <int FAMILY, int THREADS = 256>
__global__ __launch_bounds__(THREADS) void engage_observe_kernel(Params p, const float* __restrict__ actions, StepOut o) {
  extern __shared__ __attribute__((aligned(16))) uint32_t sm[];
  const Rows r{p.D, p.cfg.n_pursuers};
  const int env0 = blockIdx.x * kEPB;
  const int nvalid = min(kEPB, p.N - env0);
  TE_STAMP(p, 500, 0);
  if (threadIdx.x < kEPB) sm[r.task() * kEPB + threadIdx.x] = 0u;
  float4 my_action = make_float4(0.0f, 0.0f, 0.0f, 0.0f);
  if (threadIdx.x < kEPB && (int)threadIdx.x < nvalid) my_action = reinterpret_cast<const float4*>(actions)[env0 + threadIdx.x];
  stage_block(p, sm, r, env0);
  __syncthreads();
  TE_STAMP(p, 500, 1);
  precompute_block(p.cfg, sm, r);
  __syncthreads();
  TE_STAMP(p, 500, 2);
  if (threadIdx.x < kEPB && (int)threadIdx.x < nvalid) {
    const int lane = threadIdx.x;
    SView v{GView{p.dstate, p.estate, p.D, p.Npad, env0 + lane, r.P}, sm, lane, r, p.D, r.P, env0 + lane, true};
    const float4 a = my_action;
    if (FAMILY == FAM_STAGE01) stage01_logic(p.cfg, v, a, o);
    else if (FAMILY == FAM_STAGE02) stage02_logic(p.cfg, v, a, o);
    else level4_logic(p.cfg, v, a, o);
  }
  TE_STAMP(p, 500, 3);
  __syncthreads();
  TE_STAMP(p, 500, 4);
  if (FAMILY == FAM_LEVEL4 && p.snap) {
    const SnapRows sr{p.D, r.P};
    for (int it = threadIdx.x; it < kEPB * sr.total(); it += blockDim.x) {
      const int l = it & (kEPB - 1), w = it / kEPB;
      uint32_t v;
      if (w < 3 * p.D) v = sm[(r.obs_pos() + w) * kEPB + l];
      else if (w < sr.armed()) { const int k = (w - 3 * p.D) / r.P, s = (w - 3 * p.D) - k * r.P; v = p.dstate[((size_t)(TE_D_OBS_EULER + k) * p.D + s) * p.Npad + env0 + l]; }
      else if (w == sr.armed()) v = sm[r.anow() * kEPB + l];
      else if (w == sr.step()) v = sm[r.sstep() * kEPB + l];
      else if (w == sr.episode()) v = sm[r.sepis() * kEPB + l];
      else if (w == sr.done()) v = sm[r.done() * kEPB + l];
      else v = 0u;
      p.snap[(size_t)w * p.Npad + env0 + l] = v;
    }
    __syncthreads();
  }
  if (FAMILY == FAM_LEVEL4) {
    const uint32_t my_task = threadIdx.x < kEPB ? sm[r.task() * kEPB + threadIdx.x] : 0u;
    if (__syncthreads_or(my_task != 0u)) {
      if (threadIdx.x < kEPB) {
        const unsigned long long flagged = __ballot(my_task != 0u && (int)threadIdx.x < nvalid);
        if (my_task != 0u && (int)threadIdx.x < nvalid)
          sm[r.lcell() * kEPB + __popcll(flagged & ((1ull << threadIdx.x) - 1ull))] = threadIdx.x;
        if (threadIdx.x == 0) sm[r.lrhat() * kEPB] = (uint32_t)__popcll(flagged);
      }
      __syncthreads();
      const int n_items = (int)sm[r.lrhat() * kEPB] * p.D;
      for (int it = threadIdx.x; it < n_items; it += blockDim.x) {
        const int s = it % p.D, l = (int)sm[r.lcell() * kEPB + it / p.D];
        const uint32_t t = sm[r.task() * kEPB + l];
        SView v{GView{p.dstate, p.estate, p.D, p.Npad, env0 + l, r.P}, sm, l, r, p.D, r.P, env0 + l, false};
        level4_spawn_slot(p.cfg, v, s, (int)(t & 0xFFu), (uint32_t)v.egi(TE_E_EPISODE), (t >> 8) != 0u);
      }
      __syncthreads();
    }
    if (threadIdx.x < 192) emit_rows(p.cfg, sm, r, o.obs, env0, nvalid, threadIdx.x, 192);
    else {
      const int nprep = (int)blockDim.x - 192;
      for (int it = threadIdx.x - 192; it < kEPB * r.P; it += nprep) {
        const int l = it & (kEPB - 1), s = it / kEPB;
        if (l >= nvalid) continue;
#pragma unroll
        for (int k = 0; k < 3; ++k) p.dstate[((size_t)(TE_X_REF + k) * p.D + s) * p.Npad + env0 + l] = sm[(r.obs_pos() + k * p.D + s) * kEPB + l];
      }
      const int first = p.cfg.evaluation ? 0 : 1;
      for (int it = threadIdx.x - 192; it < kEPB * (r.P - first); it += nprep) {
        const int l = it & (kEPB - 1), s = first + it / kEPB;
        if (l >= nvalid) continue;
        SView v{GView{p.dstate, p.estate, p.D, p.Npad, env0 + l, r.P}, sm, l, r, p.D, r.P, env0 + l, sm[r.prevalid() * kEPB + l] != 0u};
        prepare_slot(p.cfg, v, s);
      }
    }
  } else {
    emit_rows(p.cfg, sm, r, o.obs, env0, nvalid, threadIdx.x, blockDim.x);
  }
  if (threadIdx.x < kEPB) {
    uint64_t dense = 0u, live = 0u; int n = 0;
    uint16_t* items = p.mixed_items + (size_t)blockIdx.x * kMixedCap;
    for (int s = 0; s < p.D; ++s)
      plan_slot<FAMILY>(items, p.dense_min, (int)threadIdx.x, s, (int)threadIdx.x < nvalid && sm[(r.armed() + s) * kEPB + threadIdx.x] != 0u, dense, n, live);
    plan_done(p, (int)blockIdx.x, (int)threadIdx.x, dense, n, live);
  }
  TE_STAMP(p, 500, 5);
  const bool lane_done = threadIdx.x < kEPB && sm[r.done() * kEPB + threadIdx.x] != 0u;
  if (o.term.lidar && __syncthreads_or(lane_done ? 1 : 0)) {
    stream_terminal_ones(p.cfg, sm, r, o.term.lidar, env0, nvalid);
    asm volatile("s_waitcnt vmcnt(0)" ::: "memory");
    __syncthreads();
  }
  TE_STAMP(p, 500, 6);
  patch_hits(p.cfg, sm, r, o.obs.lidar, o.term.lidar, env0, nvalid);
  TE_STAMP(p, 500, 7);
}

__global__ __launch_bounds__(256) void fill_ones_kernel(float* __restrict__ dst, size_t n_floats) {
  const float4 ones = make_float4(1.0f, 1.0f, 1.0f, 1.0f);
  const size_t quads = n_floats >> 2, stride = (size_t)gridDim.x * blockDim.x;
  for (size_t i = blockIdx.x * (size_t)blockDim.x + threadIdx.x; i < quads; i += stride) reinterpret_cast<float4*>(dst)[i] = ones;
  for (size_t i = (quads << 2) + blockIdx.x * (size_t)blockDim.x + threadIdx.x; i < n_floats; i += stride) dst[i] = 1.0f;
}

__global__ __launch_bounds__(256) void observe_kernel(Params p, ObsOut o) {
  extern __shared__ __attribute__((aligned(16))) uint32_t sm[];
  const Rows r{p.D, p.cfg.n_pursuers};
  const int env0 = blockIdx.x * kEPB;
  const int nvalid = min(kEPB, p.N - env0);
  if (o.lidar) stream_ones(p.cfg, o.lidar, env0, nvalid);
  stage_block(p, sm, r, env0);
  __syncthreads();
  precompute_block(p.cfg, sm, r);
  __syncthreads();
  if (threadIdx.x < kEPB && (int)threadIdx.x < nvalid) {
    const int lane = threadIdx.x;
    SView v{GView{p.dstate, p.estate, p.D, p.Npad, env0 + lane, r.P}, sm, lane, r, p.D, r.P, env0 + lane, true};
    if (v.egi(TE_E_STEP) != 0) sm[r.hitmask() * kEPB + lane] = resolve_hits(v, armed_mask(v));
  }
  __syncthreads();
  emit_rows(p.cfg, sm, r, o, env0, nvalid, threadIdx.x, blockDim.x);
  asm volatile("s_waitcnt vmcnt(0)" ::: "memory");
  __syncthreads();
  patch_hits(p.cfg, sm, r, o.lidar, nullptr, env0, nvalid);
}

__global__ void blob_to_planes(Params p, const uint32_t* __restrict__ blob) {
  const size_t ND = (size_t)p.N * p.D;
  const size_t drone_words = ND * TE_DRONE_WORDS, total = drone_words + (size_t)p.N * TE_ENV_WORDS;
  for (size_t i = blockIdx.x * (size_t)blockDim.x + threadIdx.x; i < total; i += (size_t)gridDim.x * blockDim.x) {
    if (i < drone_words) {
      size_t rec = i / TE_DRONE_WORDS; int w = (int)(i - rec * TE_DRONE_WORDS);
      int e = (int)(rec / p.D), d = (int)(rec - (size_t)e * p.D);
      p.dstate[((size_t)w * p.D + d) * p.Npad + e] = blob[i];
    } else {
      size_t j = i - drone_words; int e = (int)(j / TE_ENV_WORDS), w = (int)(j - (size_t)e * TE_ENV_WORDS);
      p.estate[(size_t)w * p.Npad + e] = blob[i];
    }
  }
}
__global__ void planes_to_blob(Params p, uint32_t* __restrict__ blob) {
  const size_t ND = (size_t)p.N * p.D;
  const size_t drone_words = ND * TE_DRONE_WORDS, total = drone_words + (size_t)p.N * TE_ENV_WORDS;
  for (size_t i = blockIdx.x * (size_t)blockDim.x + threadIdx.x; i < total; i += (size_t)gridDim.x * blockDim.x) {
    if (i < drone_words) {
      size_t rec = i / TE_DRONE_WORDS; int w = (int)(i - rec * TE_DRONE_WORDS);
      int e = (int)(rec / p.D), d = (int)(rec - (size_t)e * p.D);
      blob[i] = p.dstate[((size_t)w * p.D + d) * p.Npad + e];
    } else {
      size_t j = i - drone_words; int e = (int)(j / TE_ENV_WORDS), w = (int)(j - (size_t)e * TE_ENV_WORDS);
      blob[i] = p.estate[(size_t)w * p.Npad + e];
    }
  }
}
__global__ void init_planes(Params p) {
  for (size_t i = blockIdx.x * (size_t)blockDim.x + threadIdx.x; i < (size_t)p.D * p.Npad; i += (size_t)gridDim.x * blockDim.x)
    reinterpret_cast<float*>(p.dstate)[(size_t)(TE_D_QUAT + 3) * p.D * p.Npad + i] = 1.0f;
}
__global__ void random_actions_kernel(Params p, float* __restrict__ actions, uint64_t seed, uint64_t step_index) {
  int env = blockIdx.x * blockDim.x + threadIdx.x;
  if (env >= p.N) return;
  uint64_t g = (uint64_t)p.cfg.env_index_base + (uint64_t)env;
  U4 r = philox4x32_10((uint32_t)g, RNG_ACTION | ((uint32_t)(g >> 32) << 24), (uint32_t)step_index, (uint32_t)(step_index >> 32),
                       (uint32_t)seed, (uint32_t)(seed >> 32));
  reinterpret_cast<float4*>(actions)[env] = make_float4(-1.0f + 2.0f * u01(r.x), -1.0f + 2.0f * u01(r.y), -1.0f + 2.0f * u01(r.z), u01(r.w));
}

// ... 257 lines not shown
  }
  PolicyParams P = policy_layout(shape);
  P.base = params;
  const dim3 grid((unsigned)((n + lds.M - 1) / lds.M));
  hipLaunchKernelGGL(fn, grid, dim3(kPolThreads), (size_t)lds.words * 4, (hipStream_t)stream, P, args...);
  TE_HIP(hipGetLastError());
  return 0;
}

#define TE_POL_INSTANCES(K) \
  {{&K<2, POL_SHAPE_DEFAULT>, &K<3, POL_SHAPE_DEFAULT>}, {&K<2, POL_SHAPE_BO>, &K<3, POL_SHAPE_BO>}, {&K<2, POL_SHAPE_LEARN>, &K<3, POL_SHAPE_LEARN>}}
static_assert(POL_SHAPE_COUNT == 3, "TE_POL_INSTANCES lists every shape");
static const PolKernel<PolicyIO> kPolicyActKernels[POL_SHAPE_COUNT][2] = TE_POL_INSTANCES(policy_act_kernel);
static const PolKernel<PolicyIn, Params, int, float*> kPolicyDriveKernels[POL_SHAPE_COUNT][2] = TE_POL_INSTANCES(policy_drive_kernel);
static const PolKernel<PolicyIn, GradTileArgs> kPolicyGradKernels[POL_SHAPE_COUNT][2] = TE_POL_INSTANCES(policy_grad_tile_kernel);

static std::string shape_text(const PolShape& s) {
  std::string t = "features_dim " + std::to_string(s.F) + ", hidden";
  for (int i = 0; i < s.n_hidden; ++i) t += (i ? ", " : " ") + std::to_string(s.h[i]);
  return t;
}

static int policy_shape_id(const te_policy_shape* s, const char* fn) {
  const std::string who = std::string(fn) + ": ";
  if (!s) return fail(who + "null shape"), -1;
  std::string served = "; the served shapes, for lidar_channels 2 and 3:";
  for (int id = 0; id < POL_SHAPE_COUNT; ++id) served += (id ? " | " : " ") + shape_text(pol_shape(id, 3));
  if (s->lidar_channels != 2 && s->lidar_channels != 3)
    return fail(who + "lidar_channels must be 2 or 3, not " + std::to_string(s->lidar_channels) + served), -1;
  if (s->n_hidden < 1 || s->n_hidden > 3) return fail(who + "n_hidden must be 1, 2 or 3, not " + std::to_string(s->n_hidden) + served), -1;
  bool f_known = false;
  for (int id = 0; id < POL_SHAPE_COUNT; ++id) {
    const PolShape t = pol_shape(id, s->lidar_channels);
    if (t.F != s->features_dim) continue;
    f_known = true;
    bool same = t.n_hidden == s->n_hidden;
    for (int i = 0; same && i < t.n_hidden; ++i) same = t.h[i] == s->hidden[i];
    if (same) return id;
  }
  if (!f_known) return fail(who + "features_dim " + std::to_string(s->features_dim) + " is not served" + served), -1;
  std::string h;
  for (int i = 0; i < s->n_hidden; ++i) h += (i ? ", " : "") + std::to_string(s->hidden[i]);
  return fail(who + "hidden [" + h + "] is not served with features_dim " + std::to_string(s->features_dim) + served), -1;
}

extern "C" {

__attribute__((visibility("default"))) const char* te_last_error(void) { return g_err.c_str(); }

__attribute__((visibility("default"))) int te_create(const te_config* cfg, int32_t device_id, te_env** out) {
  if (!cfg || !out) return fail("te_create: null argument");
  if (const char* why = check_config(cfg)) return fail(why);
  const int D = cfg->n_pursuers + cfg->n_invaders;
  int ndev = 0;
  TE_HIP(hipGetDeviceCount(&ndev));
  if (ndev < 1) return fail("te_create: no HIP device visible; this library has no CPU fallback");
  if (device_id < 0 || device_id >= ndev) return fail("te_create: bad device_id");
  DeviceGuard guard(device_id);
  if (!guard.ok) return fail("te_create: hipSetDevice failed");
  te_env* e = new (std::nothrow) te_env();
  if (!e) return fail("te_create: out of host memory");
  e->device = device_id;
  e->p.dstate = nullptr; e->p.estate = nullptr; e->p.slot_mask = nullptr; e->p.live_mask = nullptr; e->p.mixed_count = nullptr; e->p.mixed_items = nullptr; e->p.stage_tab = nullptr; e->p.snap = nullptr; e->p.ring = nullptr; e->p.dbg = nullptr;
  auto bail = [&](const std::string& why) { te_destroy(e); return fail(why); };
#define TE_HIP_OR_BAIL(x)                                                                              \
  do {                                                                                                 \
    hipError_t e_ = (x);                                                                               \
    if (e_ != hipSuccess) return bail(std::string("te_create: " #x ": ") + hipGetErrorString(e_));      \
  } while (0)
  if (const char* why = plan_kernels(*cfg, &e->k)) return bail(why);
  e->family = family_of(cfg->task);
  e->p.cfg = *cfg;
  e->p.kd = derive(*cfg);
  e->p.N = cfg->n_envs; e->p.D = D; e->p.Npad = (cfg->n_envs + 63) / 64 * 64;
  e->p.dense_min = e->k.dense_min;
  hipError_t le = set_lds_limits(e->k);
  if (le != hipSuccess && e->k.engage.lds > 64 * 1024) {
    (void)hipGetLastError(); plan_kernels(*cfg, &e->k, 64 * 1024); le = set_lds_limits(e->k);
  }
  if (le != hipSuccess) return bail(std::string("te_create: this many drones per env needs more LDS than a workgroup may have: ") + hipGetErrorString(le));
  const size_t dwords = (size_t)(TE_DRONE_WORDS + TE_X_WORDS) * D * e->p.Npad, ewords = (size_t)TE_ENV_WORDS * e->p.Npad;
  if (hipMalloc(&e->p.dstate, dwords * 4) != hipSuccess || hipMalloc(&e->p.estate, ewords * 4) != hipSuccess)
    return bail("te_create: hipMalloc failed");
  if (hipMalloc(&e->p.slot_mask, (size_t)(e->p.Npad / 64) * 8) != hipSuccess || hipMalloc(&e->p.live_mask, (size_t)(e->p.Npad / 64) * 8) != hipSuccess || hipMalloc(&e->p.mixed_count, (size_t)(e->p.Npad / 64) * 4) != hipSuccess ||
      hipMalloc(&e->p.mixed_items, (size_t)(e->p.Npad / 64) * kMixedCap * sizeof(uint16_t)) != hipSuccess)
    return bail("te_create: hipMalloc failed");
  TE_HIP_OR_BAIL(hipMemsetAsync(e->p.mixed_count, 0, (size_t)(e->p.Npad / 64) * 4, nullptr));
  {
    const Rows r{D, cfg->n_pursuers};
    std::vector<uint32_t> tab((size_t)r.staged());
    for (int row = 0; row < r.staged(); ++row) tab[(size_t)row] = staged_row_offset(e->p, r, row);
    if (hipMalloc(&e->p.stage_tab, tab.size() * 4) != hipSuccess ||
        hipMemcpy(e->p.stage_tab, tab.data(), tab.size() * 4, hipMemcpyHostToDevice) != hipSuccess)
      return bail("te_create: hipMalloc failed");
  }
  if (e->k.wingman_view.fn) {
    if (hipMalloc(&e->ally_scratch, (size_t)2 * D * e->p.Npad * 4) != hipSuccess) return bail("te_create: hipMalloc failed");
  }
  if (cfg->io_location == TE_IO_HOST) {
    const size_t N = (size_t)cfg->n_envs, lw = (size_t)lidar_words(*cfg) * 4;
    const size_t blob = (N * ((size_t)D * TE_DRONE_WORDS + TE_ENV_WORDS)) * 4;
    const size_t sizes[12] = {N * 16, N * lw, N * 60, N * 16, N * 4, N * lw, N * 60, N * 16, N, N, N * 16, blob};
    size_t off[13]; off[0] = 0;
    for (int k = 0; k < 12; ++k) off[k + 1] = off[k] + ((sizes[k] + 255) & ~(size_t)255);
    if (hipMalloc(&e->hs.base, off[12]) != hipSuccess) return bail("te_create: hipMalloc failed (host I/O staging)");
    char* b = e->hs.base;
    e->hs.actions = (float*)(b + off[0]); e->hs.lidar = (float*)(b + off[1]); e->hs.inertial = (float*)(b + off[2]);
    e->hs.last_action = (float*)(b + off[3]); e->hs.reward = (float*)(b + off[4]); e->hs.t_lidar = (float*)(b + off[5]);
    e->hs.t_inertial = (float*)(b + off[6]); e->hs.t_last_action = (float*)(b + off[7]); e->hs.done = (uint8_t*)(b + off[8]);
    e->hs.mask = (uint8_t*)(b + off[9]); e->hs.info = (int32_t*)(b + off[10]); e->hs.blob = (uint32_t*)(b + off[11]);
  }
  e->p.entry_words = TE_RING_ENTRY_WORDS(D);
  if (cfg->stacked_obs && (cfg->agent_scripted || cfg->evaluation)) {
    if (hipMalloc(&e->zero_actions, (size_t)e->p.Npad * 16) != hipSuccess) return bail("te_create: hipMalloc failed");
    TE_HIP_OR_BAIL(hipMemsetAsync(e->zero_actions, 0, (size_t)e->p.Npad * 16, nullptr));
  }
  if (cfg->stacked_obs) {
    const size_t snap_bytes = (size_t)snap_words(D, cfg->n_pursuers) * e->p.Npad * 4;
    const size_t ring_bytes = (size_t)cfg->n_envs * cfg->n_pursuers * TE_RING_DEPTH * e->p.entry_words * 4;
    if (hipMalloc(&e->p.snap, snap_bytes) != hipSuccess || hipMalloc(&e->p.ring, ring_bytes) != hipSuccess)
      return bail("te_create: stacked observation buffers (ring / snapshot) could not be allocated");
    TE_HIP_OR_BAIL(hipMemsetAsync(e->p.snap, 0, snap_bytes, nullptr));
    TE_HIP_OR_BAIL(hipMemsetAsync(e->p.ring, 0, ring_bytes, nullptr));
  }
#ifdef TE_DEBUG_STAMPS
  const size_t dbg_words = 64 + 16 * (size_t)(e->p.Npad / kEPB + 1) + 4 * ((size_t)(e->p.D + kMixedWaves) * (e->p.Npad >> 6) + 4096);
  e->dbg_words = dbg_words;
  if (hipMalloc(&e->p.dbg, dbg_words * sizeof(unsigned long long)) != hipSuccess) e->p.dbg = nullptr;
  else { (void)hipMemset(e->p.dbg, 0, dbg_words * sizeof(unsigned long long)); (void)hipMemcpyToSymbol(HIP_SYMBOL(g_te_dbg), &e->p.dbg, sizeof(e->p.dbg)); }
#endif
  TE_HIP_OR_BAIL(hipMemsetAsync(e->p.dstate, 0, dwords * 4, nullptr));
  TE_HIP_OR_BAIL(hipMemsetAsync(e->p.estate, 0, ewords * 4, nullptr));
  hipLaunchKernelGGL(init_planes, dim3(256), dim3(256), 0, nullptr, e->p);
  const int blocks = (e->p.N + 255) / 256;
  launch_by_family(e->family, [&](auto fam) {
    hipLaunchKernelGGL((reset_kernel<decltype(fam)::value>), dim3(blocks), dim3(256), 0, nullptr, e->p, (const uint8_t*)nullptr);
  });
  launch_census(e, nullptr);
  TE_HIP_OR_BAIL(hipGetLastError());
  TE_HIP_OR_BAIL(hipStreamSynchronize(nullptr));
#undef TE_HIP_OR_BAIL
  *out = e;
  return 0;
}

__attribute__((visibility("default"))) int te_kernel_plan(const te_config* cfg, char* out, size_t out_bytes) {
  if (!cfg || !out) return fail("te_kernel_plan: null argument");
  KernelPlan k;
  const char* why = check_config(cfg);
  if (why || (why = plan_kernels(*cfg, &k))) return fail(why);
  std::string s = std::string("substeps=") + k.substeps[1].name + "\nsubsteps_nofill=" + k.substeps[0].name + "\nengage=" + k.engage.name + "\n" +
                  (k.ring_push.fn ? std::string("ring_push=") + k.ring_push.name + "\n" : "") + (k.stack_view.fn ? std::string("stack_view=") + k.stack_view.name + "\n" : "");
  if (k.wingman_view.fn) s += std::string("wingman_view=") + k.wingman_view.name + "+" + k.wingman_patch.name + "\n";
  else if (k.wingman_one.fn) s += std::string("wingman_view=") + k.wingman_one.name + "\n";
  if (s.size() >= out_bytes) return fail("te_kernel_plan: out_bytes too small (" + std::to_string(s.size() + 1) + " needed)");
  memcpy(out, s.c_str(), s.size() + 1);
  return 0;
}

__attribute__((visibility("default"))) void te_destroy(te_env* e) {
  if (!e) return;
  DeviceGuard guard(e->device);
  for (hipEvent_t ev : e->events) (void)hipEventDestroy(ev);
  (void)hipFree(e->p.dstate);
  (void)hipFree(e->p.estate);
  (void)hipFree(e->ally_scratch);
  (void)hipFree(e->zero_actions);
  (void)hipFree(e->hs.base); (void)hipFree(e->hs.t_gather);
  (void)hipFree(e->p.slot_mask); (void)hipFree(e->p.live_mask); (void)hipFree(e->p.mixed_count); (void)hipFree(e->p.mixed_items);
  (void)hipFree(e->p.stage_tab);
  if (e->p.snap) (void)hipFree(e->p.snap);
  if (e->p.ring) (void)hipFree(e->p.ring);
  if (e->prev_cells) (void)hipFree(e->prev_cells);
  if (e->p.dbg) (void)hipFree(e->p.dbg);
  delete e;
}

__attribute__((visibility("default"))) int te_reset(te_env* e, const uint8_t* env_mask, void* stream) {
  if (!e) return fail("te_reset: null env");
  DeviceGuard guard(e->device);
  if (host_io(e) && env_mask) {
    hipStream_t st = (hipStream_t)stream;
    TE_H2D(e->hs.mask, env_mask, (size_t)e->p.N);
    TE_HIP(hipStreamSynchronize(st));
    env_mask = e->hs.mask;
  }
  const int blocks = (e->p.N + 255) / 256;
  launch_by_family(e->family, [&](auto fam) {
    hipLaunchKernelGGL((reset_kernel<decltype(fam)::value>), dim3(blocks), dim3(256), 0, (hipStream_t)stream, e->p, env_mask);
  });
  launch_census(e, (hipStream_t)stream);
  TE_HIP(hipGetLastError());
  return 0;
}

__attribute__((visibility("default"))) int te_wingman_info(te_env* e, int32_t* wingman_info, void* stream) {
  if (!e || !wingman_info) return fail("te_wingman_info: null argument");
  if (!e->p.cfg.evaluation) return fail("te_wingman_info: per-wingman kills are only counted under cfg.evaluation (Evaluation_Task)");
  DeviceGuard guard(e->device);
  const int n = e->p.N * e->p.cfg.n_pursuers;
  hipLaunchKernelGGL(wingman_info_kernel, dim3((n + 255) / 256), dim3(256), 0, (hipStream_t)stream, e->p, wingman_info);
  TE_HIP(hipGetLastError());
  return 0;
}

static bool wingman_is_callers(const te_env* e, int wingman) {
  const te_config& c = e->p.cfg;
  if (wingman < 0 || wingman >= c.n_pursuers) return false;
  return (c.ally_policy == TE_ALLY_EXTERNAL && wingman == 1) || (((uint32_t)c.evaluation >> (8 + wingman)) & 1u) != 0u;
// ... 742 lines not shown
```

dronechase_amd/csrc/te_logic.hpp:

```cpp
#pragma once
#include "te_device.hpp"

namespace te {

constexpr int kEPB = 64;
constexpr int kMaxD = 32;
constexpr int kMaxD64 = 64;
enum Family { FAM_LEVEL4 = 0, FAM_STAGE01 = 1, FAM_STAGE02 = 2 };

struct GView {
  uint32_t* d; uint32_t* e; int D; int Npad; int env; int P;
  TE_DEV size_t ix(int w, int s) const { return ((size_t)w * D + s) * Npad + env; }
  TE_DEV float gf(int w, int s) const { return __uint_as_float(d[ix(w, s)]); }
  TE_DEV int gi(int w, int s) const { return (int)d[ix(w, s)]; }
  TE_DEV void sf(int w, int s, float v) const { d[ix(w, s)] = __float_as_uint(v); }
  TE_DEV void si(int w, int s, int v) const { d[ix(w, s)] = (uint32_t)v; }
  TE_DEV float egf(int w) const { return __uint_as_float(e[(size_t)w * Npad + env]); }
  TE_DEV int egi(int w) const { return (int)e[(size_t)w * Npad + env]; }
  TE_DEV void esf(int w, float v) const { e[(size_t)w * Npad + env] = __float_as_uint(v); }
  TE_DEV void esi(int w, int v) const { e[(size_t)w * Npad + env] = (uint32_t)v; }
};

struct Rows {
  int D, P;
// ... 67 lines not shown
  if (v.pre_valid) return (v.sm[v.at(v.r.origin())] >> s) & 1u;
  return norm(obs_pos(v, s)) < c.origin_range;
}

template <class V> TE_DEV void disarm(const V& v, int s) {
  v.si(TE_D_ARMED, s, 0);
#pragma unroll
  for (int k = 0; k < 3; ++k) { v.sf(TE_D_VEL + k, s, 0.0f); v.sf(TE_D_OMEGA + k, s, 0.0f); }
#pragma unroll
  for (int k = 0; k < 4; ++k) { v.sf(TE_D_THROTTLE + k, s, 0.0f); v.sf(TE_D_SETPOINT + k, s, 0.0f); }
}
template <class V> TE_DEV void replace_planes(const V& v, int s, V3 p) {
  v.sf(TE_D_POS, s, p.x); v.sf(TE_D_POS + 1, s, p.y); v.sf(TE_D_POS + 2, s, p.z);
  v.sf(TE_D_FORMATION, s, p.x); v.sf(TE_D_FORMATION + 1, s, p.y); v.sf(TE_D_FORMATION + 2, s, p.z);
  v.sf(TE_D_QUAT, s, 0.0f); v.sf(TE_D_QUAT + 1, s, 0.0f); v.sf(TE_D_QUAT + 2, s, 0.0f); v.sf(TE_D_QUAT + 3, s, 1.0f);
#pragma unroll
  for (int k = 0; k < 3; ++k) { v.sf(TE_D_VEL + k, s, 0.0f); v.sf(TE_D_OMEGA + k, s, 0.0f); }
}
template <class V> TE_DEV void observe_at_rest(const V& v, int s, V3 p) {
  v.sf(TE_D_OBS_POS, s, p.x); v.sf(TE_D_OBS_POS + 1, s, p.y); v.sf(TE_D_OBS_POS + 2, s, p.z);
#pragma unroll
  for (int k = 0; k < 3; ++k) { v.sf(TE_D_OBS_EULER + k, s, 0.0f); v.sf(TE_D_OBS_VEL + k, s, 0.0f); v.sf(TE_D_OBS_RATE + k, s, 0.0f); }
}
TE_DEV int max_munition_of(const te_config& c, int slot) {
  if (slot >= c.n_pursuers) return 10;
  if (c.task == TE_TASK_STAGE02) return slot == 0 ? c.munition : 10;
  return c.munition;
}
template <class V> TE_DEV void respawn_armed(const te_config& c, const V& v, int s, V3 p) {
  disarm(v, s);
  replace_planes(v, s, p);
  observe_at_rest(v, s, p);
  v.si(TE_D_ARMED, s, 1);
  v.si(TE_D_MUNITION, s, max_munition_of(c, s));
  v.si(TE_D_LAST_FIRED, s, -c.cooldown_steps);
}
TE_DEV bool gun_available(const te_config& c, int munition, int last_fired, int step) {
  return munition <= 0 || c.cooldown_steps <= step - last_fired;
}
TE_DEV void gun_state(const te_config& c, int munition, int last_fired, int step, int max_mun, float g[3]) {
  float wait = fmaxf((float)c.cooldown_steps - (float)(step - last_fired), 0.0f);
  g[0] = (float)munition / (float)(max_mun > 0 ? max_mun : 1);
  g[1] = wait / (float)c.cooldown_steps;
  g[2] = gun_available(c, munition, last_fired, step) ? 1.0f : 0.0f;
}
template <class V> TE_DEV uint32_t armed_mask(const V& v) {
  uint32_t m = 0;
  for (int s = 0; s < v.D && s < 32; ++s) m |= (v.gi(TE_D_ARMED, s) ? 1u : 0u) << s;
  return m;
}

TE_DEV void sincos_0_pi(float x, float& s, float& c) {
  TE_EXACT
  const int q = x < 0.7853981633974483f ? 0 : (x < 2.356194490192345f ? 1 : 2);
  const float y = (float)q * 2.0f;
  const float r = ((x - y * 0.78515625f) - y * 2.4187564849853515625e-4f) - y * 3.77489497744594108e-8f;
  const float z = r * r;
  const float sr = r + r * z * (-1.6666654611e-1f + z * (8.3321608736e-3f + z * -1.9515295891e-4f));
  const float cr = 1.0f - 0.5f * z + z * z * (4.166664568298827e-2f + z * (-1.388731625493765e-3f + z * 2.443315711809948e-5f));
  s = q == 0 ? sr : (q == 1 ? cr : -sr);
  c = q == 0 ? cr : (q == 1 ? -sr : -cr);
}
TE_DEV V3 level4_position(const te_config& c, float r, float u_theta, float u_phi) {
  TE_EXACT
  float theta = u_theta * kPi;
  float lower = fminf(c.born_min_z, r);
  float min_phi = 0.5f * kPi - x_asin(lower * rcp(r));
  float phi = (r >= c.born_min_z) ? min_phi + u_phi * (0.5f * kPi - min_phi) : u_phi * (0.5f * kPi);
  float sph, cph, sth, cth;
  sincos_0_pi(phi, sph, cph); sincos_0_pi(theta, sth, cth);
  return V3{r * sph * cth, r * sph * sth, r * cph};
}
TE_DEV V3 stage02_position(float r, float r_max, float u_r, float u_theta, float u_phi) {
  TE_EXACT
  if (r > r_max) r_max = r;
  float radius = r + u_r * (r_max - r);
  float theta = u_theta * 2.0f * kPi, phi = u_phi * kPi * 0.5f;
  float sph, cph, sth, cth;
  sincosf(phi, &sph, &cph); sincosf(theta, &sth, &cth);
  return V3{radius * sph * cth, radius * sph * sth, radius * cph};
}

TE_DEV int invaders_in_round(const te_config& c, int round) { return min((round - 1) * c.invaders_per_round + c.initial_invaders, c.n_invaders); }
__host__ __device__ __forceinline__ bool all_scripted(const te_config& c) { return c.evaluation != 0 || c.agent_scripted != 0; }
template <class V> TE_DEV void set_snap_mask(const V& v, uint64_t m) { v.esi(TE_E_SNAP_MASK, (int)(uint32_t)m); v.esi(TE_E_SNAP_MASK_HI, (int)(uint32_t)(m >> 32)); }
template <class V> TE_DEV uint64_t get_snap_mask(const V& v) { return (uint64_t)(uint32_t)v.egi(TE_E_SNAP_MASK) | ((uint64_t)(uint32_t)v.egi(TE_E_SNAP_MASK_HI) << 32); }
template <class V> TE_DEV int closest_invader(const V& v, uint64_t mask, int p, float& dmin) {
  int best = -1; dmin = 0.0f;
  for (int j = v.P; j < v.D; ++j) {
    if (!((mask >> j) & 1u)) continue;
    float d = pi_dist(v, p, j);
    if (best < 0 || d < dmin) { best = j; dmin = d; }
  }
  return best;
}
template <class V> TE_DEV int closest_pursuer(const V& v, uint64_t mask, int j) {
  int best = -1; float bd = 0.0f;
  for (int p = 0; p < v.P; ++p) {
    if (!((mask >> p) & 1u)) continue;
    float d = pi_dist(v, p, j);
    if (best < 0 || d < bd) { best = p; bd = d; }
  }
  return best;
}
template <class V> TE_DEV int closest_ally(const V& v, uint64_t mask, int p) {
  if (!((mask >> p) & 1u) || __popc((uint32_t)mask & ((1u << v.P) - 1u)) <= 1) return -1;
  V3 me = obs_pos(v, p);
  int best = -1; float bd = 0.0f;
  for (int a = 0; a < v.P; ++a) {
    if (a == p || !((mask >> a) & 1u)) continue;
    float d = dist(obs_pos(v, a), me);
    if (best < 0 || d < bd) { best = a; bd = d; }
  }
  return best;
}

TE_DEV void x_cmd_toward(V3 from, V3 to, float speed, float out[3]) {
  TE_EXACT
  const float dx = to.x - from.x, dy = to.y - from.y, dz = to.z - from.z;
  const float n = sqrtf(xfma(dz, dz, xfma(dy, dy, dx * dx)));
  const float inv = n > 0.0f ? 1.0f / n : 1.0f;
  const float ux = dx * inv, uy = dy * inv, uz = dz * inv;
  const float m = sqrtf(xfma(uz, uz, xfma(uy, uy, ux * ux)));
  const float inv2 = 1.0f / (m > 0.0f ? m : 1.0f);
  out[0] = speed * (ux * inv2); out[1] = speed * (uy * inv2); out[2] = speed * (uz * inv2);
}
TE_DEV void cmd_toward(V3 from, V3 to, float speed, float out[3]) { x_cmd_toward(from, to, speed, out); }
TE_DEV bool inside_cone(V3 p, V3 apex, V3 base, float degrees) {
  V3 ab = sub(base, apex), ap = sub(p, apex);
  float nab = norm(ab), nap = norm(ap);
  if (nap > nab) return false;
  float cosang = (ap.x * ab.x + ap.y * ab.y + ap.z * ab.z) / (nap * nab);
  return acosf(cosang) * (180.0f / kPi) <= 0.5f * degrees;
}
template <class V> TE_DEV bool building_path_clear(const te_config& c, const V& v, uint32_t mask, V3 me, float degrees) {
  if (!c.kamikaze_cone_check) return false;
  V3 b{c.building_position[0], c.building_position[1], c.building_position[2]};
  for (int p = 0; p < c.n_pursuers; ++p)
    if (((mask >> p) & 1u) && inside_cone(obs_pos(v, p), me, b, degrees)) return false;
  return true;
}
template <class V> TE_DEV int kamikaze_update(const te_config& c, const V& v, uint32_t S, int state, V3 me, float out[3]) {
  const int Pn = c.n_pursuers;
  const uint32_t pursuer_bits = S & ((1u << Pn) - 1u);
  int next = state;
  if (state == TE_NAV_WAIT) {
    if (building_path_clear(c, v, S, me, 60.0f)) next = TE_NAV_COLLIDE_BUILDING;
    else if (pursuer_bits) next = TE_NAV_COLLIDE_WINGMAN;
    out[0] = out[1] = out[2] = 0.0f;
  } else if (state == TE_NAV_COLLIDE_WINGMAN) {
    if (!pursuer_bits) next = TE_NAV_COLLIDE_BUILDING;
    int best = -1; float bd = 0.0f; V3 target{0, 0, 0};
    for (int p = 0; p < Pn; ++p) {
      if (!((S >> p) & 1u)) continue;
      const V3 pp = obs_pos(v, p);
      const float d = dist(pp, me);
      if (best < 0 || d < bd) { best = p; bd = d; target = pp; }
    }
    cmd_toward(me, target, c.invader_speed, out);
  } else {
    if (!building_path_clear(c, v, S, me, 45.0f)) next = TE_NAV_COLLIDE_WINGMAN;
    cmd_toward(me, V3{c.building_position[0], c.building_position[1], c.building_position[2]}, c.invader_speed, out);
  }
  return next;
}
TE_DEV bool driven_externally(const te_config& c, int s) {
// ... 574 lines not shown
```

Baseline: 916.6 million.

## Precompute per-chunk wake mask and park slot-0 state in LDS to cut registers

The previous step now computes a per-chunk wake mask of invader slots that may spawn next round and stores it next to the live mask as one 16-byte record. Slot waves read this mask to decide early exit instead of loading the round and doing a ballot at kernel start. Slot 0's IMU, action and counters are moved from registers into extra LDS rows, and waves-per-EU is pinned to 8, aiming to lower register pressure and raise occupancy. This costs more LDS per block, a wider mask buffer, and extra mask computation in the producing kernels.

```diff
diff --git a/dronechase_amd/csrc/te_engage.hpp b/dronechase_amd/csrc/te_engage.hpp
--- a/dronechase_amd/csrc/te_engage.hpp
+++ b/dronechase_amd/csrc/te_engage.hpp
@@ -243,8 +243,7 @@
   uint32_t armed_w[DM];
   int mun[PM], lf[PM];
   float fx[PM], fy[PM], fz[PM];
-  const uint32_t* __restrict__ lm32 = reinterpret_cast<const uint32_t*>(p.live_mask);
-  const uint64_t live = (uint64_t)__builtin_amdgcn_readfirstlane(lm32[2 * blockIdx.x]) | ((uint64_t)__builtin_amdgcn_readfirstlane(lm32[2 * blockIdx.x + 1]) << 32);
+  const uint64_t live = chunk_masks(p, (int)blockIdx.x).live;
 #pragma unroll
   for (int s = 0; s < DM; ++s) {
     px[s] = py[s] = pz[s] = 0.0f; armed_w[s] = 0u;
@@ -640,7 +639,8 @@
     uint64_t dense = 0u, live = 0u; int n = 0;
     uint16_t* items = p.mixed_items + (size_t)blockIdx.x * kMixedCap;
     for (int s = 0; s < D; ++s) plan_slot_l4<void>(items, p.dense_min, lane, s, valid && ((armed_post >> s) & one) != 0, dense, n, live);
-    if (lane == 0) { p.slot_mask[blockIdx.x] = dense; p.mixed_count[blockIdx.x] = (uint32_t)n; p.live_mask[blockIdx.x] = live; }
+    const uint64_t wake = wake_mask_of(c, D, valid, round);
+    if (lane == 0) plan_store(p, (int)blockIdx.x, dense, (uint32_t)n, live, wake);
   }
   TE_ESTAMP(10, 0);
   TE_ESTAMP(11, 1);
@@ -885,7 +885,7 @@
   {
     uint64_t dense = 0u;
     for (int s = 0; s < D; ++s) if (__ballot(valid && ((A >> s) & 1u))) dense |= (uint64_t)1 << s;
-    if (lane == 0) { p.slot_mask[blockIdx.x] = dense; p.mixed_count[blockIdx.x] = 0u; p.live_mask[blockIdx.x] = dense; }
+    if (lane == 0) plan_store(p, (int)blockIdx.x, dense, 0u, dense, dense);
   }
 }
 
@@ -969,8 +969,8 @@
   {
     uint64_t dense = 0u;
     for (int s = 0; s < 3; ++s) if (__ballot(valid && ((A >> s) & 1u))) dense |= (uint64_t)1 << s;
-    if (lane == 0) { p.slot_mask[blockIdx.x] = dense; p.mixed_count[blockIdx.x] = 0u; p.live_mask[blockIdx.x] = dense; }
-  }
-}
-
-}
+    if (lane == 0) plan_store(p, (int)blockIdx.x, dense, 0u, dense, dense);
+  }
+}
+
+}
diff --git a/dronechase_amd/csrc/te_engage_slots.hpp b/dronechase_amd/csrc/te_engage_slots.hpp
--- a/dronechase_amd/csrc/te_engage_slots.hpp
+++ b/dronechase_amd/csrc/te_engage_slots.hpp
@@ -17,8 +17,10 @@
   TE_DEV int npos(int k, int s) const { return 4 + (5 + k) * D + s; }
   TE_DEV int prec(int q) const { return 4 + 8 * D + q; }
   TE_DEV int prec2(int q) const { return 4 + 8 * D + 2 * q; }
+  TE_DEV int w0(int k) const { return 4 + 8 * D + 2 * P + k; }
 };
-__host__ __device__ inline int slot_lds_rows(int D, int P) { return 4 + 8 * D + 2 * P; }
+constexpr int kSlotParked = 17;
+__host__ __device__ inline int slot_lds_rows(int D, int P) { return 4 + 8 * D + 2 * P + kSlotParked; }
 enum : uint32_t { SLOT_HIT = 1u << 8, SLOT_EXPLODE = 1u << 9, SLOT_SUICIDE = 1u << 10 };
 
 #define TE_SLOT_BARRIER() asm volatile("s_waitcnt lgkmcnt(0)\n\ts_barrier" ::: "memory")
@@ -28,12 +30,25 @@
     if (wait) asm volatile("s_waitcnt vmcnt(0) lgkmcnt(0)" ::: "memory");                                                 \
     if (p.dbg && s < 2 && lane == 0) p.dbg[64 + blockIdx.x * 16 + s * 8 + (idx)] = __builtin_amdgcn_s_memrealtime();     \
   } while (0)
+#define TE_WLIFE_BASE(p) (64 + 16 * (size_t)((p).Npad / 64 + 1) + 4 * ((size_t)((p).D + kMixedWaves) * ((p).Npad >> 6) + 4096))
+#define TE_WLIFE_BEGIN const unsigned long long wl_t0_ = __builtin_amdgcn_s_memrealtime();
+#define TE_WLIFE_END(kind)                                                                                                \
+  do {                                                                                                                    \
+    if (p.dbg && lane == 0) {                                                                                             \
+      unsigned long long* r_ = p.dbg + TE_WLIFE_BASE(p) + 4 * ((size_t)blockIdx.x * kSlotWaves + s);                      \
+      r_[0] = wl_t0_; r_[1] = __builtin_amdgcn_s_memrealtime();                                                           \
+      r_[2] = (unsigned long long)__builtin_amdgcn_s_getreg((31 << 11) | 4) | ((unsigned long long)__builtin_amdgcn_s_getreg((31 << 11) | 20) << 32); \
+      r_[3] = (kind);                                                                                                     \
+    }                                                                                                                     \
+  } while (0)
 #else
 #define TE_WSTAMP(idx, wait) do {} while (0)
+#define TE_WLIFE_BEGIN
+#define TE_WLIFE_END(kind) do {} while (0)
 #endif
 
 template <int DM>
-__global__ __launch_bounds__(DM * 64) __attribute__((amdgpu_waves_per_eu(6, 10))) void engage_slots_kernel(Params p, const float* __restrict__ actions, StepOut o) {
+__global__ __launch_bounds__(DM * 64) __attribute__((amdgpu_waves_per_eu(8, 8))) void engage_slots_kernel(Params p, const float* __restrict__ actions, StepOut o) {
   TE_EXACT
   extern __shared__ uint32_t sm[];
   const te_config& c = p.cfg;
@@ -51,33 +66,31 @@
   auto L = [&](int row) -> uint32_t& { return sm[row * 64 + lane]; };
   auto Lf = [&](int row) { return __uint_as_float(sm[row * 64 + lane]); };
   auto Lor = [&](int row, uint32_t v) { __hip_atomic_fetch_or(&sm[row * 64 + lane], v, __ATOMIC_RELAXED, __HIP_MEMORY_SCOPE_WORKGROUP); };
+  TE_WLIFE_BEGIN
   TE_WSTAMP(0, 0);
 
-  const uint32_t* __restrict__ lm32 = reinterpret_cast<const uint32_t*>(p.live_mask);
-  const uint32_t live = (uint32_t)__builtin_amdgcn_readfirstlane(lm32[2 * blockIdx.x]) & all_bits;
+  const ChunkMasks cm = chunk_masks(p, (int)blockIdx.x);
+  const uint32_t live = (uint32_t)cm.live & all_bits, wake = (uint32_t)cm.wake & all_bits;
   const bool mine_live = is_p || ((live >> s) & 1u);
-  auto next_round_of = [&](int r) { return r + (r < c.n_rounds ? 1 : c.n_rounds); };
-  auto may_be_spawned = [&](int slot, int r) { const int i = slot - P; return i < invaders_in_round(c, next_round_of(r)) || i < invaders_in_round(c, 1); };
-  if (!mine_live) {
-    const int r = (int)io.le(TE_E_ROUND);
-    if (__ballot(valid && may_be_spawned(s, r)) == 0ull) return;
-  }
+  if (!mine_live && !((wake >> s) & 1u)) { TE_WLIFE_END(1); return; }
   float mx = io.ldf(TE_D_OBS_POS, s), my = io.ldf(TE_D_OBS_POS + 1, s), mz = io.ldf(TE_D_OBS_POS + 2, s);
   const uint32_t marmed_w = io.ld(TE_D_ARMED, s);
   const V3 apos{io.ldf(TE_D_OBS_POS, 0), io.ldf(TE_D_OBS_POS + 1, 0), io.ldf(TE_D_OBS_POS + 2, 0)};
-  float ag[9];
+  float ag[3];
 #pragma unroll
   for (int k = 0; k < 3; ++k) ag[k] = io.ldf(TE_D_OBS_EULER + k, 0);
-#pragma unroll
-  for (int k = 3; k < 9; ++k) ag[k] = 0.0f;
   const uint32_t w_step = io.le(TE_E_STEP), w_max_step = io.le(TE_E_MAX_STEP), w_round = io.le(TE_E_ROUND), w_episode = io.le(TE_E_EPISODE);
-  uint32_t w_last_dist = 0u, w_ak = 0u, w_lk = 0u, w_dd = 0u;
-  float4 act = make_float4(0.0f, 0.0f, 0.0f, 0.0f);
+  uint32_t w0w[kSlotParked - 3];
+#pragma unroll
+  for (int k = 0; k < kSlotParked - 3; ++k) w0w[k] = 0u;
   if (s == 0) {
 #pragma unroll
-    for (int k = 3; k < 9; ++k) ag[k] = io.ldf(TE_D_OBS_EULER + k, 0);
-    w_last_dist = io.le(TE_E_LAST_DIST); w_ak = io.le(TE_E_AGENT_KILLS); w_lk = io.le(TE_E_ALLIES_KILLS); w_dd = io.le(TE_E_DEADS);
-    if (valid) act = reinterpret_cast<const float4*>(actions)[env];
+    for (int k = 3; k < 9; ++k) w0w[k - 3] = io.ld(TE_D_OBS_EULER + k, 0);
+    w0w[6] = io.le(TE_E_LAST_DIST); w0w[7] = io.le(TE_E_AGENT_KILLS); w0w[8] = io.le(TE_E_ALLIES_KILLS); w0w[9] = io.le(TE_E_DEADS);
+    if (valid) {
+      const float4 a4 = reinterpret_cast<const float4*>(actions)[env];
+      w0w[10] = __float_as_uint(a4.x); w0w[11] = __float_as_uint(a4.y); w0w[12] = __float_as_uint(a4.z); w0w[13] = __float_as_uint(a4.w);
+    }
   }
   uint32_t w_mun = 0u, w_lf = 0u; float fx = 0.0f, fy = 0.0f, fz = 0.0f;
   if (is_p) {
@@ -92,10 +105,19 @@
   int max_step = (int)w_max_step, round = (int)w_round;
   uint32_t episode = w_episode;
   int mun = (int)w_mun, lf = (int)w_lf;
-  const float last_dist = __uint_as_float(w_last_dist);
-  int agent_kills = (int)w_ak, allies_kills = (int)w_lk, deads = (int)w_dd;
   if (!mine_live) { mx = my = mz = 0.0f; }
   TE_WSTAMP(1, 1);
+  if (s == 0) {
+#pragma unroll
+    for (int k = 0; k < 3; ++k) L(R.w0(k)) = __float_as_uint(ag[k]);
+#pragma unroll
+    for (int k = 0; k < kSlotParked - 3; ++k) L(R.w0(3 + k)) = w0w[k];
+  }
+  auto parked_imu = [&](float a9[9]) {
+#pragma unroll
+    for (int k = 0; k < 9; ++k) a9[k] = Lf(R.w0(k));
+  };
+  auto parked_action = [&]() { return make_float4(Lf(R.w0(13)), Lf(R.w0(14)), Lf(R.w0(15)), Lf(R.w0(16))); };
 
   const uint32_t a_me = (mine_live && marmed_w != zero && valid) ? 1u : 0u;
   {
@@ -191,14 +213,16 @@
 
   auto pos_of = [&](int t) { return V3{__uint_as_float(sm[R.pos(0, t) * 64 + lane]), __uint_as_float(sm[R.pos(1, t) * 64 + lane]), __uint_as_float(sm[R.pos(2, t) * 64 + lane])}; };
   if (s == 0) {
+    const float4 act = parked_action();
+    const float last_dist = Lf(R.w0(9));
+    const int agent_kills = (int)L(R.w0(10)) + agent_shots, allies_kills = (int)L(R.w0(11)) + ally_shots, deads = (int)L(R.w0(12)) + exploded;
     if (valid) {
       io.stef(TE_E_LAST_ACTION + 0, act.x); io.stef(TE_E_LAST_ACTION + 1, act.y); io.stef(TE_E_LAST_ACTION + 2, act.z); io.stef(TE_E_LAST_ACTION + 3, act.w);
       io.ste(TE_E_STEP, (uint32_t)step);
       io.ste(TE_E_SNAP_MASK, S); io.ste(TE_E_SNAP_MASK_HI, 0u);
     }
-    agent_kills += agent_shots; allies_kills += ally_shots; deads += exploded;
     if (to_terminal) {
-      if (o.term.inertial) inertial_row_regs(c, o.term.inertial + (size_t)env * TE_OBS_INERTIAL_WORDS, mx, my, mz, ag, mun, lf, step);
+      if (o.term.inertial) { float a9[9]; parked_imu(a9); inertial_row_regs(c, o.term.inertial + (size_t)env * TE_OBS_INERTIAL_WORDS, mx, my, mz, a9, mun, lf, step); }
       if (o.term.last_action) reinterpret_cast<float4*>(o.term.last_action)[env] = act;
     }
     float reward = 0.0f, cur_dist = last_dist;
@@ -222,7 +246,7 @@
       cur_dist = fdist(apos, tp);
       const bool ready = gs[2] == 1.0f || gs[0] == 0.0f;
       float bonus = 0.0f, penalty = 0.0f;
-      if (0.01f < last_dist - cur_dist && ready) bonus += c.approach_bonus_gain * fnorm(V3{ag[3], ag[4], ag[5]});
+      if (0.01f < last_dist - cur_dist && ready) bonus += c.approach_bonus_gain * fnorm(V3{Lf(R.w0(3)), Lf(R.w0(4)), Lf(R.w0(5))});
       const float score = ready ? -cur_dist : cur_dist * (2.0f * gs[1] - 1.0f);
       if (agent_shots > 0 || agent_suicided > 0) bonus += (float)(agent_shots + agent_suicided) * 1000.0f;
       if (ally_shots > 0 || pursuer_suicided > 0) bonus += 0.5f * (float)(ally_shots + pursuer_suicided) * 1000.0f;
@@ -267,9 +291,6 @@
       for (int k = 0; k < 4; ++k) io.ste(TE_E_LAST_ACTION + k, 0u);
       io.ste(TE_E_SNAP_MASK, snap_mask); io.ste(TE_E_SNAP_MASK_HI, 0u);
     }
-    act = make_float4(0.0f, 0.0f, 0.0f, 0.0f);
-#pragma unroll
-    for (int k = 0; k < 9; ++k) ag[k] = 0.0f;
     task = 1u | (1u << 8);
   }
   if (task != 0u) {
@@ -280,9 +301,8 @@
     if (reset && is_p) { mun = max_munition_of(c, s); lf = -c.cooldown_steps; fx = mx; fy = my; fz = mz; }
   }
   if (s == 0 && __ballot(task != 0u) != 0ull) {
-    for (uint32_t m = inv_bits & ~live; m; m &= m - 1u) {
+    for (uint32_t m = inv_bits & ~live & ~wake; m; m &= m - 1u) {
       const int k2 = __ffs((int)m) - 1;
-      if (__ballot(valid && may_be_spawned(k2, (int)w_round)) != 0ull) continue;
       if (task != 0u) io.st(TE_D_NAV_STATE, k2, (uint32_t)TE_NAV_WAIT);
     }
   }
@@ -301,8 +321,14 @@
     else if (own && !to_terminal) pv[(size_t)(__popc(owners & ((1u << s) - 1u)) + 1) * p.Npad] = (uint16_t)cj;
   }
   if (s == 0) {
-    if (o.obs.inertial && valid) inertial_row_regs(c, o.obs.inertial + (size_t)env * TE_OBS_INERTIAL_WORDS, mx, my, mz, ag, mun, lf, step);
-    if (valid && o.obs.last_action) reinterpret_cast<float4*>(o.obs.last_action)[env] = act;
+    if (o.obs.inertial && valid) {
+      float a9[9];
+      parked_imu(a9);
+#pragma unroll
+      for (int k = 0; k < 9; ++k) a9[k] = to_terminal ? 0.0f : a9[k];
+      inertial_row_regs(c, o.obs.inertial + (size_t)env * TE_OBS_INERTIAL_WORDS, mx, my, mz, a9, mun, lf, step);
+    }
+    if (valid && o.obs.last_action) reinterpret_cast<float4*>(o.obs.last_action)[env] = to_terminal ? make_float4(0.0f, 0.0f, 0.0f, 0.0f) : parked_action();
   }
   if (is_p && valid) {
     int first_skipped = -1;
@@ -337,6 +363,7 @@
   if (s >= 1 || s == writer) {
     uint64_t dense = 0u, livem = 0u; int n = 0;
     uint16_t* items = p.mixed_items + (size_t)blockIdx.x * kMixedCap;
+    const uint64_t wakem = s == writer ? wake_mask_of(c, D, valid, round) : 0u;
     const int k_last = s == writer ? D - 1 : s;
     for (int k = 0; k <= k_last; ++k) {
       const bool a = valid && ((armed_post >> k) & 1u) != 0u;
@@ -348,10 +375,11 @@
       if (k == s && a) items[n + (int)__builtin_amdgcn_mbcnt_hi((uint32_t)(b >> 32), __builtin_amdgcn_mbcnt_lo((uint32_t)b, 0u))] = (uint16_t)(lane | (k << 8));
       n += cnt;
     }
-    if (s == writer && lane == 0) { p.slot_mask[blockIdx.x] = dense; p.mixed_count[blockIdx.x] = (uint32_t)n; p.live_mask[blockIdx.x] = livem; }
+    if (s == writer && lane == 0) plan_store(p, (int)blockIdx.x, dense, (uint32_t)n, livem, wakem);
   }
   TE_WSTAMP(6, 0);
   TE_WSTAMP(7, 1);
+  TE_WLIFE_END(2);
 }
 
 struct MultiSlotRows {
@@ -398,20 +426,16 @@
   auto Lor = [&](int row, uint32_t v) { __hip_atomic_fetch_or(&sm[row * 64 + lane], v, __ATOMIC_RELAXED, __HIP_MEMORY_SCOPE_WORKGROUP); };
   TE_WSTAMP(0, 0);
 
-  const uint32_t* __restrict__ lm32 = reinterpret_cast<const uint32_t*>(p.live_mask);
-  const M live = (WIDE ? (M)((uint64_t)(uint32_t)__builtin_amdgcn_readfirstlane(lm32[2 * blockIdx.x]) | ((uint64_t)(uint32_t)__builtin_amdgcn_readfirstlane(lm32[2 * blockIdx.x + 1]) << 32))
-                       : (M)(uint32_t)__builtin_amdgcn_readfirstlane(lm32[2 * blockIdx.x])) & all_bits;
-  auto next_round_of = [&](int r) { return r + (r < c.n_rounds ? 1 : c.n_rounds); };
-  auto may_be_spawned = [&](int slot, int r) { const int i = slot - P; return i < invaders_in_round(c, next_round_of(r)) || i < invaders_in_round(c, 1); };
+  const ChunkMasks cm = chunk_masks(p, (int)blockIdx.x);
+  const M live = (M)cm.live & all_bits, wake = (M)cm.wake & all_bits;
   bool mine_live[SPW]; bool any_live = is_p;
 #pragma unroll
   for (int u = 0; u < SPW; ++u) { mine_live[u] = has[u] && ((u == 0 && is_p) || ((live >> (sl[u] & kSh)) & one) != 0); any_live = any_live || mine_live[u]; }
   if (!any_live) {
-    const int r = (int)io.le(TE_E_ROUND);
     bool maybe = false;
 #pragma unroll
-    for (int u = 0; u < SPW; ++u) maybe = maybe || (has[u] && may_be_spawned(sl[u], r));
-    if (__ballot(valid && maybe) == 0ull) return;
+    for (int u = 0; u < SPW; ++u) maybe = maybe || (has[u] && ((wake >> (sl[u] & kSh)) & one) != 0);
+    if (!maybe) return;
   }
   float mx[SPW], my[SPW], mz[SPW]; uint32_t marmed_w[SPW];
 #pragma unroll
@@ -729,7 +753,7 @@
       bool stayed = wv < P;
       for (int u2 = 0; u2 < SPW && !stayed; ++u2) {
         const int s2 = wv + u2 * W;
-        if (s2 < D) stayed = ((live >> s2) & one) != 0 || __ballot(valid && may_be_spawned(s2, (int)w_round)) != 0ull;
+        if (s2 < D) stayed = (((live | wake) >> s2) & one) != 0;
       }
       if (stayed) continue;
       if (task != 0u) io.st(TE_D_NAV_STATE, k2, (uint32_t)TE_NAV_WAIT);
@@ -796,6 +820,7 @@
     for (int u = 1; u < SPW; ++u) if (has[u]) top = sl[u];
     uint64_t dense = 0u, livem = 0u; int n = 0;
     uint16_t* items = p.mixed_items + (size_t)blockIdx.x * kMixedCap;
+    const uint64_t wakem = s == writer ? wake_mask_of(c, D, valid, round) : 0u;
     const int k_last = s == writer ? D - 1 : top;
     for (int k = 0; k <= k_last; ++k) {
       const bool a = valid && ((armed_post >> k) & one) != 0;
@@ -810,7 +835,7 @@
       if (own && a) items[n + (int)__builtin_amdgcn_mbcnt_hi((uint32_t)(b >> 32), __builtin_amdgcn_mbcnt_lo((uint32_t)b, 0u))] = (uint16_t)(lane | (k << 8));
       n += cnt;
     }
-    if (s == writer && lane == 0) { p.slot_mask[blockIdx.x] = dense; p.mixed_count[blockIdx.x] = (uint32_t)n; p.live_mask[blockIdx.x] = livem; }
+    if (s == writer && lane == 0) plan_store(p, (int)blockIdx.x, dense, (uint32_t)n, livem, wakem);
   }
   TE_WSTAMP(6, 0);
   TE_WSTAMP(7, 1);
@@ -1035,7 +1060,7 @@
     const uint32_t armed_post = to_terminal ? all_bits : ((A & pur_bits) | (valid ? inv_bits : 0u));
     uint64_t dense = 0u;
     for (int k = 0; k < D; ++k) if (__ballot(valid && ((armed_post >> k) & 1u))) dense |= (uint64_t)1 << k;
-    if (lane == 0) { p.slot_mask[blockIdx.x] = dense; p.mixed_count[blockIdx.x] = 0u; p.live_mask[blockIdx.x] = dense; }
+    if (lane == 0) plan_store(p, (int)blockIdx.x, dense, 0u, dense, dense);
   }
 }
 
diff --git a/dronechase_amd/csrc/te_env.hip b/dronechase_amd/csrc/te_env.hip
--- a/dronechase_amd/csrc/te_env.hip
+++ b/dronechase_amd/csrc/te_env.hip
@@ -405,8 +405,10 @@
   if (a) items[n + (int)__builtin_amdgcn_mbcnt_hi((uint32_t)(b >> 32), __builtin_amdgcn_mbcnt_lo((uint32_t)b, 0u))] = (uint16_t)(lane | (s << 8));
   n += cnt;
 }
-TE_DEV void plan_done(const Params& p, int chunk, int lane, uint64_t dense, int n, uint64_t live) {
-  if (lane == 0) { p.slot_mask[chunk] = dense; p.mixed_count[chunk] = (uint32_t)n; p.live_mask[chunk] = live; }
+template <int FAMILY>
+TE_DEV void plan_done(const Params& p, int chunk, int lane, bool valid, int round, uint64_t dense, int n, uint64_t live) {
+  const uint64_t wake = FAMILY == FAM_LEVEL4 ? wake_mask_of(p.cfg, p.D, valid, round) : live;
+  if (lane == 0) plan_store(p, chunk, dense, (uint32_t)n, live, wake);
 }
 template <int FAMILY>
 __global__ __launch_bounds__(64) void census_kernel(Params p) {
@@ -414,7 +416,7 @@
   uint64_t dense = 0u, live = 0u; int n = 0;
   uint16_t* items = p.mixed_items + (size_t)chunk * kMixedCap;
   for (int s = 0; s < p.D; ++s) plan_slot<FAMILY>(items, p.dense_min, l, s, env < p.N && p.dstate[((size_t)TE_D_ARMED * p.D + s) * p.Npad + env] != 0u, dense, n, live);
-  plan_done(p, chunk, l, dense, n, live);
+  plan_done<FAMILY>(p, chunk, l, env < p.N, env < p.N ? (int)p.estate[(size_t)TE_E_ROUND * p.Npad + env] : 0, dense, n, live);
 }
 __global__ __launch_bounds__(256) void prepare_commands_kernel(Params p) {
   int env = blockIdx.x * 256 + threadIdx.x;
@@ -552,7 +554,7 @@
     uint16_t* items = p.mixed_items + (size_t)blockIdx.x * kMixedCap;
     for (int s = 0; s < p.D; ++s)
       plan_slot<FAMILY>(items, p.dense_min, (int)threadIdx.x, s, (int)threadIdx.x < nvalid && sm[(r.armed() + s) * kEPB + threadIdx.x] != 0u, dense, n, live);
-    plan_done(p, (int)blockIdx.x, (int)threadIdx.x, dense, n, live);
+    plan_done<FAMILY>(p, (int)blockIdx.x, (int)threadIdx.x, (int)threadIdx.x < nvalid, (int)sm[(r.env() + TE_E_ROUND) * kEPB + threadIdx.x], dense, n, live);
   }
   TE_STAMP(p, 500, 5);
   const bool lane_done = threadIdx.x < kEPB && sm[r.done() * kEPB + threadIdx.x] != 0u;
@@ -976,7 +978,7 @@
   const size_t dwords = (size_t)(TE_DRONE_WORDS + TE_X_WORDS) * D * e->p.Npad, ewords = (size_t)TE_ENV_WORDS * e->p.Npad;
   if (hipMalloc(&e->p.dstate, dwords * 4) != hipSuccess || hipMalloc(&e->p.estate, ewords * 4) != hipSuccess)
     return bail("te_create: hipMalloc failed");
-  if (hipMalloc(&e->p.slot_mask, (size_t)(e->p.Npad / 64) * 8) != hipSuccess || hipMalloc(&e->p.live_mask, (size_t)(e->p.Npad / 64) * 8) != hipSuccess || hipMalloc(&e->p.mixed_count, (size_t)(e->p.Npad / 64) * 4) != hipSuccess ||
+  if (hipMalloc(&e->p.slot_mask, (size_t)(e->p.Npad / 64) * 8) != hipSuccess || hipMalloc(&e->p.live_mask, (size_t)(e->p.Npad / 64) * 16) != hipSuccess || hipMalloc(&e->p.mixed_count, (size_t)(e->p.Npad / 64) * 4) != hipSuccess ||
       hipMalloc(&e->p.mixed_items, (size_t)(e->p.Npad / 64) * kMixedCap * sizeof(uint16_t)) != hipSuccess)
     return bail("te_create: hipMalloc failed");
   TE_HIP_OR_BAIL(hipMemsetAsync(e->p.mixed_count, 0, (size_t)(e->p.Npad / 64) * 4, nullptr));
@@ -1018,7 +1020,7 @@
     TE_HIP_OR_BAIL(hipMemsetAsync(e->p.ring, 0, ring_bytes, nullptr));
   }
 #ifdef TE_DEBUG_STAMPS
-  const size_t dbg_words = 64 + 16 * (size_t)(e->p.Npad / kEPB + 1) + 4 * ((size_t)(e->p.D + kMixedWaves) * (e->p.Npad >> 6) + 4096);
+  const size_t dbg_words = TE_WLIFE_BASE(e->p) + 4 * (size_t)kSlotWaves * (e->p.Npad >> 6);
   e->dbg_words = dbg_words;
   if (hipMalloc(&e->p.dbg, dbg_words * sizeof(unsigned long long)) != hipSuccess) e->p.dbg = nullptr;
   else { (void)hipMemset(e->p.dbg, 0, dbg_words * sizeof(unsigned long long)); (void)hipMemcpyToSymbol(HIP_SYMBOL(g_te_dbg), &e->p.dbg, sizeof(e->p.dbg)); }
diff --git a/dronechase_amd/csrc/te_logic.hpp b/dronechase_amd/csrc/te_logic.hpp
--- a/dronechase_amd/csrc/te_logic.hpp
+++ b/dronechase_amd/csrc/te_logic.hpp
@@ -173,6 +173,27 @@
 }
 
 TE_DEV int invaders_in_round(const te_config& c, int round) { return min((round - 1) * c.invaders_per_round + c.initial_invaders, c.n_invaders); }
+TE_DEV int next_round_of(const te_config& c, int r) { return r + (r < c.n_rounds ? 1 : c.n_rounds); }
+TE_DEV int spawn_reach(const te_config& c, int r) { return max(invaders_in_round(c, next_round_of(c, r)), invaders_in_round(c, 1)); }
+TE_DEV bool may_be_spawned(const te_config& c, int slot, int r) { return slot - c.n_pursuers < spawn_reach(c, r); }
+TE_DEV uint64_t wake_mask_of(const te_config& c, int D, bool valid, int round) {
+  const int reach = valid ? c.n_pursuers + spawn_reach(c, round) : 0;
+  uint64_t wake = 0u;
+  for (int s = 0; s < D; ++s)
+    if (__ballot(s < reach) != 0ull) wake |= (uint64_t)1 << s;
+  return wake;
+}
+TE_DEV void plan_store(const Params& p, int chunk, uint64_t dense, uint32_t n, uint64_t live, uint64_t wake) {
+  p.slot_mask[chunk] = dense; p.mixed_count[chunk] = n;
+  *reinterpret_cast<uint4*>(p.live_mask + 2 * (size_t)chunk) = make_uint4((uint32_t)live, (uint32_t)(live >> 32), (uint32_t)wake, (uint32_t)(wake >> 32));
+}
+struct ChunkMasks { uint64_t live, wake; };
+TE_DEV ChunkMasks chunk_masks(const Params& p, int chunk) {
+  const uint4 w = *reinterpret_cast<const uint4*>(p.live_mask + 2 * (size_t)chunk);
+  const uint32_t l0 = (uint32_t)__builtin_amdgcn_readfirstlane((int)w.x), l1 = (uint32_t)__builtin_amdgcn_readfirstlane((int)w.y);
+  const uint32_t w0 = (uint32_t)__builtin_amdgcn_readfirstlane((int)w.z), w1 = (uint32_t)__builtin_amdgcn_readfirstlane((int)w.w);
+  return ChunkMasks{(uint64_t)l0 | ((uint64_t)l1 << 32), (uint64_t)w0 | ((uint64_t)w1 << 32)};
+}
 __host__ __device__ __forceinline__ bool all_scripted(const te_config& c) { return c.evaluation != 0 || c.agent_scripted != 0; }
 template <class V> TE_DEV void set_snap_mask(const V& v, uint64_t m) { v.esi(TE_E_SNAP_MASK, (int)(uint32_t)m); v.esi(TE_E_SNAP_MASK_HI, (int)(uint32_t)(m >> 32)); }
 template <class V> TE_DEV uint64_t get_snap_mask(const V& v) { return (uint64_t)(uint32_t)v.egi(TE_E_SNAP_MASK) | ((uint64_t)(uint32_t)v.egi(TE_E_SNAP_MASK_HI) << 32); }
```

Measured after the change: 908.4 million. Within noise of the previous version (-0.9%).
